# Sujit-O/pykg2vec

Measured on AMD Instinct MI355X. Metric: scored triples/sec (train) + test-triples ranked/sec, FB15k TransE d=100, higher is better.
Workload: dtype f32

## Files before the change

### include/kge_hip.h

```cpp
#ifndef KGE_HIP_H
#define KGE_HIP_H

#include <stddef.h>
#include <stdint.h>

#ifdef __cplusplus
extern "C" {
#endif

#define KGE_ABI_VERSION 3
#define KGE_MAX_TABLES 12

enum kge_model {
    KGE_TRANSE = 0,
    KGE_TRANSH = 1,
    KGE_TRANSD = 2,
    KGE_ROTATE = 3,
    KGE_RESCAL = 4,
    KGE_NTN = 5,
    KGE_DISTMULT = 6,
    KGE_COMPLEX = 7,
    KGE_ANALOGY = 8,
    KGE_TRANSM = 9,
    KGE_CP = 10,
    KGE_SIMPLE = 11,
    KGE_SIMPLE_IGNR = 12,
    KGE_QUATE = 13,
    KGE_TRANSR = 14,
    KGE_SLM = 15,
    KGE_SME = 16,
    KGE_SME_BL = 17,
    KGE_KG2E = 18,
    KGE_HOLE = 19,
    KGE_OCTONIONE = 20
};


#define KGE_FLAG_L1 1u

enum kge_optimizer { KGE_OPT_SGD = 0, KGE_OPT_ADAM = 1, KGE_OPT_ADAGRAD = 2, KGE_OPT_RMSPROP = 3,
                     KGE_OPT_GRADIENT = 4  };
enum kge_reg { KGE_REG_NONE = 0, KGE_REG_F2 = 1, KGE_REG_N3 = 2, KGE_REG_N3_ABS = 3, KGE_REG_ID_F2 = 4, KGE_REG_ID_N3 = 5 };

typedef struct kge_model_desc {
    int32_t model;
    uint32_t flags;
    int64_t tot_entity;
    int64_t tot_relation;
    int32_t dim;
    int32_t rel_dim;
    float margin;
    float phase_scale;
    const float* tables[KGE_MAX_TABLES];
    float* grads[KGE_MAX_TABLES];
} kge_model_desc;

int kge_abi_version(void);
const char* kge_last_error(void);

int kge_set_debug(int32_t check_ids);
int kge_set_switch(const char* name, int32_t value);
int kge_get_debug(void);
int kge_check_ids(const int64_t* ids, int64_t n, int64_t bound, void* stream);
size_t kge_filter_csr_workspace_bytes(int64_t n_known, int64_t n_queries);
int kge_filter_csr_count(const int64_t* known, int64_t n_known, const int64_t* queries, int64_t n_queries, int64_t tot_entity,
                         int64_t tot_relation, void* workspace, size_t workspace_bytes, int64_t* tail_off, int64_t* head_off,
                         int64_t* totals, void* stream);
int kge_filter_csr_fill(const int64_t* queries, int64_t n_queries, int64_t n_known, const void* workspace, const int64_t* tail_off,
                        const int64_t* head_off, int32_t* tail_ids, int32_t* head_ids, void* stream);

#define KGE_TOPK_MAX 1024
size_t kge_topk_workspace_bytes(int64_t nq, int64_t n_cand, int masked);
int kge_topk_rows(const void* scores, int dtype, int64_t nq, int64_t n_cand, int64_t row_stride, int32_t k, int largest,
                  const int64_t* skip_off, const int32_t* skip_ids, const int64_t* keep, void* workspace, size_t workspace_bytes,
                  int32_t* out_ids, void* out_scores, int32_t* out_count, void* stream);

#define KGE_CAND_CHUNK 64
size_t kge_rank_candidates_workspace_bytes(int64_t n, int64_t n_lists, int64_t n_cand_ids);
int kge_rank_candidates(const kge_model_desc* m, const int64_t* triples, int64_t n, int32_t side, const int64_t* list_of_query,
                        const int64_t* cand_off, const int32_t* cand_ids, int64_t n_lists, const int64_t* skip_off,
                        const int32_t* skip_ids, void* workspace, size_t workspace_bytes, int32_t* counts, void* stream);
int kge_rank_lists_from_scores(const void* scores, int dtype, const void* truth_scores, const int64_t* seg_off, int64_t n,
                               const uint8_t* flags, int largest, int32_t* counts, void* stream);

#define KGE_REL_CHUNK 64
size_t kge_rank_relations_workspace_bytes(int64_t n);
int kge_rank_relations(const kge_model_desc* m, const int64_t* triples, int64_t n, const int64_t* skip_off, const int32_t* skip_ids,
                       void* workspace, size_t workspace_bytes, int32_t* counts, void* stream);
size_t kge_relation_csr_workspace_bytes(int64_t n_known, int64_t n_queries);
int kge_relation_csr_count(const int64_t* known, int64_t n_known, const int64_t* queries, int64_t n_queries, int64_t tot_entity,
                           int64_t tot_relation, void* workspace, size_t workspace_bytes, int64_t* rel_off, int64_t* total, void* stream);
int kge_relation_csr_fill(const int64_t* queries, int64_t n_queries, int64_t n_known, const void* workspace, const int64_t* rel_off,
                          int32_t* rel_ids, void* stream);

int kge_debug_marker(int32_t tag, void* stream);

size_t kge_workspace_bytes(const kge_model_desc* m, int64_t n);

int kge_score_forward(const kge_model_desc* m, const int64_t* h, const int64_t* r, const int64_t* t,
                      int64_t n, float* scores, void* workspace, size_t workspace_bytes, void* stream);

int kge_score_backward(const kge_model_desc* m, const int64_t* h, const int64_t* r, const int64_t* t,
                       int64_t n, const float* dscore, void* workspace, size_t workspace_bytes, void* stream);

int kge_rescal_normalize(float* ent, int64_t tot_entity, float* rel, int64_t tot_relation, int32_t k,
                         void* stream);
size_t kge_rescal_normalize_scratch_bytes(int64_t tot_relation, int32_t k);
int kge_rescal_normalize_ws(float* ent , int64_t tot_entity, float* rel, int64_t tot_relation,
                            int32_t k, void* scratch, size_t scratch_bytes, void* stream);

int kge_train_pairwise_hinge(const kge_model_desc* m,
                             const int64_t* ph, const int64_t* pr, const int64_t* pt,
                             const int64_t* nh, const int64_t* nr, const int64_t* nt,
                             int64_t n, float margin, void* workspace, size_t workspace_bytes,
                             float* loss, void* stream);

int kge_train_pairwise_hinge_sampled(const kge_model_desc* m, const int64_t* triples, const int64_t* perm,
                                     int64_t start, int64_t n, const float* bern_prob, const uint64_t* slots,
                                     int64_t n_slots, uint64_t seed, uint64_t offset, const int64_t* dev_cursor,
                                     float margin, float* loss, void* stream);

int kge_train_pairwise_selfadv(const kge_model_desc* m,
                               const int64_t* ph, const int64_t* pr, const int64_t* pt,
                               const int64_t* nh, const int64_t* nr, const int64_t* nt,
                               int64_t n_pos, int32_t neg_rate, float alpha, float* workspace,
                               float* loss, void* stream);

int kge_train_pairwise_selfadv_sampled(const kge_model_desc* m, const int64_t* triples, const int64_t* perm,
                                       int64_t start, int64_t n_pos, int32_t neg_rate, float alpha,
                                       const float* bern_prob, const uint64_t* slots, int64_t n_slots,
                                       uint64_t seed, uint64_t offset, const int64_t* dev_cursor,
                                       float* loss, void* stream);

int kge_train_pointwise_logistic(const kge_model_desc* m, const int64_t* h, const int64_t* r,
                                 const int64_t* t, const int64_t* y, int64_t n,
                                 int32_t bundle ,
                                 float lmbda, int32_t reg_type, float* loss, void* stream);

int kge_train_pointwise_logistic_sampled(const kge_model_desc* m, const int64_t* triples, const int64_t* perm,
                                         int64_t start, int64_t n_pos, int32_t neg_rate, const float* bern_prob,
                                         const uint64_t* slots, int64_t n_slots, uint64_t seed, uint64_t offset,
                                         const int64_t* dev_cursor, float lmbda, int32_t reg_type, float* loss,
                                         void* stream);

int kge_optimizer_step(int32_t kind, float* param, float* grad, float* state1, float* state2,
                       int64_t numel, float lr, int64_t step, int32_t zero_grad,
                       const float* dev_hyper ,
                       void* stream);

int kge_optimizer_step_rows(int32_t kind, float* param, float* grad, float* state1, float* state2, int64_t rows, int32_t dim,
                            float lr, int64_t step, int32_t zero_grad, int32_t normalize, const float* dev_hyper,
                            const uint32_t* touched_rows, uint32_t* touched_clear, void* stream);

int kge_rescal_pair_step(const kge_model_desc* m, const int64_t* ph, const int64_t* pr, const int64_t* pt, const int64_t* nh,
                         const int64_t* nt, int64_t n, float margin, void* workspace, size_t workspace_bytes, float* loss,
                         uint32_t* touched_rows, void* stream);
int kge_rescal_pair_step_ok(const kge_model_desc* m, int64_t n);

typedef struct kge_rescal_stage {
    float* gstage;
    float* dsv;
    int32_t* count;
    int32_t* bucket;
    int32_t* head;
    int32_t* next;
    int32_t cap;
} kge_rescal_stage;
int kge_rescal_stage_ok(const kge_model_desc* m, int64_t n);
int kge_rescal_pair_step_staged(const kge_model_desc* m, const int64_t* ph, const int64_t* pr, const int64_t* pt, const int64_t* nh,
                                const int64_t* nt, int64_t n, float margin, void* workspace, size_t workspace_bytes, float* loss,
                                uint32_t* touched_rows, const kge_rescal_stage* stage, void* stream);
int kge_optimizer_step_rows_staged(int32_t kind, float* param, float* grad, float* state1, float* state2, int64_t rows, int32_t dim,
                                   float lr, int64_t step, int32_t normalize, const float* dev_hyper, const uint32_t* touched_rows,
                                   uint32_t* touched_clear, const kge_rescal_stage* stage, void* stream);

int kge_l2norm_reg(const float* param, float* grad, int64_t numel, float lmbda, float* scratch, float* loss,
                   void* stream);

size_t kge_eval_workspace_bytes(const kge_model_desc* m, int64_t n);
int kge_eval_ranks(const kge_model_desc* m, const int64_t* triples, int64_t n,
                   const int64_t* tail_off, const int32_t* tail_ids,
                   const int64_t* head_off, const int32_t* head_ids,
                   void* workspace, size_t workspace_bytes, int32_t* ranks, void* stream);

size_t kge_eval_grouped_workspace_bytes(const kge_model_desc* m, int64_t n, int64_t n_groups);
int kge_eval_ranks_grouped(const kge_model_desc* m, const int64_t* triples, int64_t n,
                           const int32_t* group_of_triple, const int64_t* group_rel, int64_t n_groups,
                           const int32_t* qblocks, int64_t n_qblocks,
                           const int64_t* tail_off, const int32_t* tail_ids,
                           const int64_t* head_off, const int32_t* head_ids,
                           void* workspace, size_t workspace_bytes, int32_t* ranks, void* stream);

int kge_eval_ranks_ties(const kge_model_desc* m, const int64_t* triples, int64_t n, const int64_t* tail_off,
                        const int32_t* tail_ids, const int64_t* head_off, const int32_t* head_ids, void* workspace,
                        size_t workspace_bytes, int32_t* ranks, int32_t* ties, void* stream);
int kge_eval_ranks_grouped_ties(const kge_model_desc* m, const int64_t* triples, int64_t n, const int32_t* group_of_triple,
                                const int64_t* group_rel, int64_t n_groups, const int32_t* qblocks, int64_t n_qblocks,
                                const int64_t* tail_off, const int32_t* tail_ids, const int64_t* head_off,
                                const int32_t* head_ids, void* workspace, size_t workspace_bytes, int32_t* ranks, int32_t* ties,
                                void* stream);

int kge_eval_sweep_scores(const kge_model_desc* m, const int64_t* triples, int64_t n,
                          void* workspace, size_t workspace_bytes, float* scores, void* stream);

int kge_eval_sweep_scores_side(const kge_model_desc* m, const int64_t* triples, int64_t n, int side,
                               void* workspace, size_t workspace_bytes, float* scores, void* stream);

int kge_rank_from_scores(const float* scores, int64_t nq, int64_t tot_entity, const int64_t* truth,
                         const int64_t* off, const int32_t* ids, int32_t* rank, int32_t* frank, void* stream);

int kge_triple_set_build(const int64_t* triples, int64_t n, uint64_t* slots, int64_t n_slots, void* stream);
int kge_corrupt(const int64_t* ph, const int64_t* pr, const int64_t* pt, int64_t n_pos, int32_t neg_rate,
                int64_t tot_entity, const float* bern_prob ,
                const uint64_t* slots, int64_t n_slots, uint64_t seed, uint64_t offset,
                int64_t* nh, int64_t* nr, int64_t* nt, void* stream);

int kge_sample_batch(const int64_t* triples, const int64_t* perm, int64_t start, int64_t n_pos, int32_t neg_rate,
                     int64_t tot_entity, const float* bern_prob, const uint64_t* slots, int64_t n_slots,
                     uint64_t seed, uint64_t offset, int32_t layout,
                     int64_t* o0, int64_t* o1, int64_t* o2, int64_t* o3, int64_t* o4, int64_t* o5,
                     const int64_t* dev_cursor ,
                     void* stream);

int kge_step_advance(int64_t* dev_cursor, float* dev_hyper, int64_t batch_stride, int64_t n_batches,
                     int64_t draws_per_batch, float lr, void* stream);

int kge_optimizer_step_rownorm_ok(int64_t rows, int64_t dim);
int kge_optimizer_step_rownorm(int32_t kind, float* param, float* grad, float* state1, float* state2, int64_t rows, int64_t dim, float lr,
                               int64_t step, int32_t zero_grad, const float* dev_hyper, void* scratch, size_t scratch_bytes,
                               const int64_t* dev_cursor, int64_t* next_cursor, float* next_hyper, int64_t batch_stride,
                               int64_t n_batches, int64_t draws_per_batch, void* stream);

int kge_optimizer_step_rows_rownorm(int32_t kind, float* param, float* grad, float* state1, float* state2, int64_t rows, int32_t dim,
                                    float* wparam, float* wgrad, float* wstate1, float* wstate2, int64_t wrows, int64_t wdim,
                                    float lr, int64_t step, int32_t zero_grad, int32_t normalize, const float* dev_hyper,
                                    const uint32_t* touched_rows, uint32_t* touched_clear, const kge_rescal_stage* stage,
                                    void* scratch, size_t scratch_bytes, const int64_t* dev_cursor, int64_t* next_cursor,
                                    float* next_hyper, int64_t batch_stride, int64_t n_batches, int64_t draws_per_batch, void* stream);

int kge_optimizer_step_advance(int32_t kind, float* param, float* grad, float* state1, float* state2,
                               int64_t numel, float lr, int32_t zero_grad,
                               const float* dev_hyper, const int64_t* dev_cursor,
                               int64_t* next_cursor, float* next_hyper,
                               int64_t batch_stride, int64_t n_batches, int64_t draws_per_batch, void* stream);

#define KGE_PULL_BUCKET 16
typedef struct kge_pull_lists {
    int32_t* pc;
    int32_t* count;
    int32_t* bucket;
    int32_t* head;
    int32_t* next;
    int32_t* sdesc;
    int32_t* dbucket;
} kge_pull_lists;
typedef struct kge_pull_direction {
    void* codes;
    float* recs;
    int64_t n_pairs;
    int32_t lists_without_descriptors;
} kge_pull_direction;
int kge_pull_direction_bytes(int32_t dim, int32_t l1, int64_t n_pairs, size_t* codes_bytes, size_t* recs_bytes);
int kge_pull_partial_stride(int32_t dim);
int kge_pull_hat_stride(int32_t dim);
int kge_pull_groups_per_block(int32_t dim);
int kge_row_norms(const float* table, int64_t rows, int32_t dim, float* norms, float* normalised, void* stream);
int kge_pull_sample(const int32_t* pairs, const int32_t* inv, int64_t n, int64_t tot_entity, const float* bern_prob,
                    const uint64_t* slots, int64_t n_slots, uint64_t seed, uint64_t offset, const int64_t* dev_cursor,
                    const kge_pull_lists* out, void* stream);
int kge_pull_lists_explicit(const int32_t* pairs, const int32_t* inv, const int64_t* nh, const int64_t* nt, int64_t n,
                            const kge_pull_lists* out, void* stream);
int kge_pull_step(const kge_model_desc* m, float* const tables_out[2], const float* const hat_in[2], float* const hat_out[2],
                  const float* norm_in, float* norm_out,
                  float* const state1[2], float* const state2[2], const int32_t* pairs, const kge_pull_lists* lists,
                  const int32_t* items, int64_t n_items, const uint32_t* dense_skip, const int32_t* inc, float* partials, const int32_t* multi,
                  int64_t n_multi, float margin, int32_t optimizer, float lr, int64_t step, const float* dev_hyper,
                  int32_t reset_lists, const int32_t* next_pairs, const int32_t* next_inv, int64_t next_n, const float* bern_prob,
                  const uint64_t* slots, int64_t n_slots, uint64_t seed, uint64_t next_offset, const kge_pull_lists* next_lists,
// ... 429 lines not shown
```

### pykg2vec_amd/_lib.py

```python
import ctypes
import os

_HERE = os.path.dirname(os.path.abspath(__file__))
LIB_PATH = os.environ.get("KGE_HIP_LIB", os.path.join(_HERE, "libkge_hip.so"))

KGE_MAX_TABLES = 12
ABI_VERSION = 3

(TRANSE, TRANSH, TRANSD, ROTATE, RESCAL, NTN, DISTMULT, COMPLEX, ANALOGY, TRANSM, CP, SIMPLE, SIMPLE_IGNR,
 QUATE, TRANSR, SLM, SME, SME_BL, KG2E, HOLE, OCTONIONE) = range(21)
FLAG_L1 = 1
OPT_SGD, OPT_ADAM, OPT_ADAGRAD, OPT_RMSPROP = range(4)
REG_NONE, REG_F2, REG_N3, REG_N3_ABS, REG_ID_F2, REG_ID_N3 = range(6)
LOSS_SLOTS, LOSS_STRIDE = 32, 32

c_i64p = ctypes.c_void_p


class ModelDesc(ctypes.Structure):
    _fields_ = [
        ("model", ctypes.c_int32),
        ("flags", ctypes.c_uint32),
        ("tot_entity", ctypes.c_int64),
        ("tot_relation", ctypes.c_int64),
# ... 197 lines not shown
_SIGNATURES = {
    **_conv_1n_signatures("interacte", InteracteDesc),
    **_conv_1n_signatures("acre", AcreDesc),
    **_conv_1n_signatures("hyper", HyperDesc),
    **_conv_1n_signatures("conve", ConveDesc, has_side=True),
    "kge_proje_body_forward_workspace_bytes": (ctypes.c_size_t, [_PJD, ctypes.c_int64]),
    "kge_proje_body_forward": (ctypes.c_int, [_PJD, ctypes.c_void_p, ctypes.c_void_p, ctypes.c_int64, ctypes.c_int32, ctypes.c_void_p,
                                              ctypes.c_void_p, ctypes.c_size_t, ctypes.c_void_p]),
    "kge_proje_body_backward_workspace_bytes": (ctypes.c_size_t, [_PJD, ctypes.c_int64]),
    "kge_proje_body_backward": (ctypes.c_int, [_PJD, ctypes.c_void_p, ctypes.c_void_p, ctypes.c_int64, ctypes.c_int32, ctypes.c_void_p,
                                               ctypes.c_void_p, ctypes.c_size_t, ctypes.c_void_p]),
    "kge_proje_label_loss_workspace_bytes": (ctypes.c_size_t, [ctypes.c_int64, ctypes.c_int32, ctypes.c_int64, ctypes.c_int64]),
    "kge_proje_label_loss": (ctypes.c_int, [ctypes.c_void_p, ctypes.c_int64, ctypes.c_int32, ctypes.c_void_p, ctypes.c_int64, ctypes.c_void_p,
                                            ctypes.c_void_p, ctypes.c_int64, ctypes.c_void_p, ctypes.c_int64, ctypes.c_void_p,
                                            ctypes.c_size_t] + [ctypes.c_void_p] * 4),
    "kge_proje_train_workspace_bytes": (ctypes.c_size_t, [_PJD] + [ctypes.c_int64] * 4),
    "kge_proje_train": (ctypes.c_int, [_PJD] + [ctypes.c_void_p] * 3 + [ctypes.c_int64, ctypes.c_void_p, ctypes.c_void_p, ctypes.c_int64,
                                                                      ctypes.c_void_p, ctypes.c_void_p, ctypes.c_int64, ctypes.c_void_p,
                                                                      ctypes.c_int64, ctypes.c_float, ctypes.c_void_p, ctypes.c_size_t,
                                                                      ctypes.c_void_p, ctypes.c_void_p]),
    "kge_proje_eval_ranks_workspace_bytes": (ctypes.c_size_t, [_PJD, ctypes.c_int64]),
    "kge_proje_eval_ranks": (ctypes.c_int, [_PJD, ctypes.c_void_p, ctypes.c_int64] + [ctypes.c_void_p] * 4
                             + [ctypes.c_void_p, ctypes.c_size_t, ctypes.c_void_p, ctypes.c_void_p, ctypes.c_void_p]),
    "kge_tucker_saved_floats": (ctypes.c_size_t, [_TKD, ctypes.c_int64]),
    "kge_tucker_body_forward_workspace_bytes": (ctypes.c_size_t, [_TKD, ctypes.c_int64]),
    "kge_tucker_body_forward": (ctypes.c_int, [_TKD, ctypes.c_void_p, ctypes.c_void_p, ctypes.c_int64, ctypes.c_void_p, ctypes.c_void_p,
                                               ctypes.c_void_p, ctypes.c_size_t, ctypes.c_void_p]),
    "kge_tucker_body_backward_workspace_bytes": (ctypes.c_size_t, [_TKD, ctypes.c_int64]),
    "kge_tucker_body_backward": (ctypes.c_int, [_TKD, ctypes.c_void_p, ctypes.c_void_p, ctypes.c_int64, ctypes.c_void_p, ctypes.c_void_p,
                                                ctypes.c_void_p, ctypes.c_size_t, ctypes.c_void_p]),
    "kge_tucker_train_bce_workspace_bytes": (ctypes.c_size_t, [_TKD, ctypes.c_int64, ctypes.c_int64, ctypes.c_int64]),
    "kge_tucker_train_bce": (ctypes.c_int, [_TKD] + [ctypes.c_void_p] * 3 + [ctypes.c_int64, ctypes.c_void_p, ctypes.c_void_p, ctypes.c_int64,
                                                                           ctypes.c_void_p, ctypes.c_void_p, ctypes.c_int64, ctypes.c_float,
                                                                           ctypes.c_void_p, ctypes.c_size_t, ctypes.c_void_p, ctypes.c_void_p]),
    "kge_tucker_eval_ranks_workspace_bytes": (ctypes.c_size_t, [_TKD, ctypes.c_int64]),
    "kge_tucker_eval_ranks": (ctypes.c_int, [_TKD, ctypes.c_void_p, ctypes.c_int64] + [ctypes.c_void_p] * 4
                              + [ctypes.c_void_p, ctypes.c_size_t, ctypes.c_void_p, ctypes.c_void_p, ctypes.c_void_p]),
    "kge_convkb_collapse_workspace_bytes": (ctypes.c_size_t, [_CKB]),
    "kge_convkb_collapse": (ctypes.c_int, [_CKB, ctypes.c_void_p, ctypes.c_void_p, ctypes.c_size_t, ctypes.c_void_p]),
    "kge_convkb_score_forward_workspace_bytes": (ctypes.c_size_t, [_CKB, ctypes.c_int64]),
    "kge_convkb_score_forward": (ctypes.c_int, [_CKB] + [ctypes.c_void_p] * 3 + [ctypes.c_int64, ctypes.c_void_p, ctypes.c_void_p,
                                                                               ctypes.c_size_t, ctypes.c_void_p]),
    "kge_convkb_score_backward_workspace_bytes": (ctypes.c_size_t, [_CKB, ctypes.c_int64]),
    "kge_convkb_score_backward": (ctypes.c_int, [_CKB] + [ctypes.c_void_p] * 3 + [ctypes.c_int64, ctypes.c_void_p, ctypes.c_void_p,
                                                                                ctypes.c_size_t, ctypes.c_void_p]),
    "kge_convkb_train_logistic_workspace_bytes": (ctypes.c_size_t, [_CKB, ctypes.c_int64]),
    "kge_convkb_train_logistic": (ctypes.c_int, [_CKB] + [ctypes.c_void_p] * 4 + [ctypes.c_int64, ctypes.c_int32, ctypes.c_void_p,
                                                                                ctypes.c_size_t, ctypes.c_void_p, ctypes.c_void_p]),
    "kge_convkb_train_logistic_sampled_workspace_bytes": (ctypes.c_size_t, [_CKB, ctypes.c_int64, ctypes.c_int32]),
    "kge_convkb_train_logistic_sampled": (ctypes.c_int, [_CKB, ctypes.c_void_p, ctypes.c_void_p, ctypes.c_int64, ctypes.c_int64,
                                                         ctypes.c_int32, ctypes.c_void_p, ctypes.c_void_p, ctypes.c_int64,
                                                         ctypes.c_uint64, ctypes.c_uint64, ctypes.c_void_p, ctypes.c_void_p,
                                                         ctypes.c_size_t, ctypes.c_void_p, ctypes.c_void_p]),
    "kge_convkb_eval_ranks_workspace_bytes": (ctypes.c_size_t, [_CKB, ctypes.c_int64]),
    "kge_convkb_eval_ranks": (ctypes.c_int, [_CKB, ctypes.c_void_p, ctypes.c_int64] + [ctypes.c_void_p] * 4
                              + [ctypes.c_void_p, ctypes.c_size_t, ctypes.c_void_p, ctypes.c_void_p]),
    "kge_convkb_sweep_scores_side_workspace_bytes": (ctypes.c_size_t, [_CKB, ctypes.c_int64]),
    "kge_murp_score_forward": (ctypes.c_int, [_MRP] + [ctypes.c_void_p] * 3 + [ctypes.c_int64, ctypes.c_void_p, ctypes.c_void_p]),
    "kge_murp_score_backward": (ctypes.c_int, [_MRP] + [ctypes.c_void_p] * 3 + [ctypes.c_int64, ctypes.c_void_p, ctypes.c_void_p]),
    "kge_murp_train_bce": (ctypes.c_int, [_MRP] + [ctypes.c_void_p] * 4 + [ctypes.c_int64, ctypes.c_void_p, ctypes.c_void_p]),
    "kge_murp_rsgd_step": (ctypes.c_int, [_MRP, ctypes.c_double, ctypes.c_int32, ctypes.c_void_p]),
    "kge_murp_eval_ranks_workspace_bytes": (ctypes.c_size_t, [_MRP, ctypes.c_int64]),
    "kge_murp_eval_ranks": (ctypes.c_int, [_MRP, ctypes.c_void_p, ctypes.c_int64] + [ctypes.c_void_p] * 4
                            + [ctypes.c_void_p, ctypes.c_size_t, ctypes.c_void_p, ctypes.c_void_p, ctypes.c_void_p]),
    "kge_murp_sweep_scores_side_workspace_bytes": (ctypes.c_size_t, [_MRP, ctypes.c_int64]),
    "kge_murp_sweep_scores_side": (ctypes.c_int, [_MRP, ctypes.c_void_p, ctypes.c_int64, ctypes.c_int32, ctypes.c_void_p,
                                                  ctypes.c_size_t, ctypes.c_void_p, ctypes.c_void_p]),
    "kge_convkb_sweep_scores_side": (ctypes.c_int, [_CKB, ctypes.c_void_p, ctypes.c_int64, ctypes.c_int32, ctypes.c_void_p,
                                                    ctypes.c_size_t, ctypes.c_void_p, ctypes.c_void_p]),
    "kge_staged_step_bytes": (ctypes.c_size_t, []),
    "kge_train_pairwise_selfadv_sampled_staged": (ctypes.c_int, [ctypes.POINTER(ModelDesc), ctypes.c_void_p, ctypes.c_void_p, ctypes.c_int64,
                                                                  ctypes.c_int64, ctypes.c_int32, ctypes.c_float, ctypes.c_void_p,
                                                                  ctypes.c_void_p, ctypes.c_int64, ctypes.c_uint64, ctypes.c_uint64,
                                                                  ctypes.POINTER(StagedStep), ctypes.c_void_p, ctypes.c_void_p]),
    "kge_train_pointwise_logistic_sampled_staged": (ctypes.c_int, [ctypes.POINTER(ModelDesc), ctypes.c_void_p, ctypes.c_void_p, ctypes.c_int64,
                                                                    ctypes.c_int64, ctypes.c_int32, ctypes.c_void_p, ctypes.c_void_p,
                                                                    ctypes.c_int64, ctypes.c_uint64, ctypes.c_uint64, ctypes.c_float,
                                                                    ctypes.c_int32, ctypes.POINTER(StagedStep), ctypes.c_void_p,
                                                                    ctypes.c_void_p]),
    "kge_optimizer_step_staged": (ctypes.c_int, [ctypes.c_int32, ctypes.POINTER(StagedStep), ctypes.c_float, ctypes.c_int64, ctypes.c_void_p]),
    "kge_abi_version": (ctypes.c_int, []),
    "kge_set_debug": (ctypes.c_int, [ctypes.c_int32]),
    "kge_set_switch": (ctypes.c_int, [ctypes.c_char_p, ctypes.c_int32]),
    "kge_get_debug": (ctypes.c_int, []),
    "kge_check_ids": (ctypes.c_int, [ctypes.c_void_p, ctypes.c_int64, ctypes.c_int64, ctypes.c_void_p]),
    "kge_debug_marker": (ctypes.c_int, [ctypes.c_int32, ctypes.c_void_p]),
    "kge_filter_csr_workspace_bytes": (ctypes.c_size_t, [ctypes.c_int64, ctypes.c_int64]),
    "kge_filter_csr_count": (ctypes.c_int, [ctypes.c_void_p, ctypes.c_int64, ctypes.c_void_p, ctypes.c_int64, ctypes.c_int64, ctypes.c_int64,
                                            ctypes.c_void_p, ctypes.c_size_t, ctypes.c_void_p, ctypes.c_void_p, ctypes.c_void_p, ctypes.c_void_p]),
    "kge_filter_csr_fill": (ctypes.c_int, [ctypes.c_void_p, ctypes.c_int64, ctypes.c_int64, ctypes.c_void_p, ctypes.c_void_p, ctypes.c_void_p,
                                           ctypes.c_void_p, ctypes.c_void_p, ctypes.c_void_p]),
    "kge_topk_workspace_bytes": (ctypes.c_size_t, [ctypes.c_int64, ctypes.c_int64, ctypes.c_int]),
    "kge_topk_rows": (ctypes.c_int, [ctypes.c_void_p, ctypes.c_int, ctypes.c_int64, ctypes.c_int64, ctypes.c_int64, ctypes.c_int32, ctypes.c_int,
                                     ctypes.c_void_p, ctypes.c_void_p, ctypes.c_void_p, ctypes.c_void_p, ctypes.c_size_t,
                                     ctypes.c_void_p, ctypes.c_void_p, ctypes.c_void_p, ctypes.c_void_p]),
    "kge_rank_candidates_workspace_bytes": (ctypes.c_size_t, [ctypes.c_int64, ctypes.c_int64, ctypes.c_int64]),
    "kge_rank_candidates": (ctypes.c_int, [ctypes.POINTER(ModelDesc), ctypes.c_void_p, ctypes.c_int64, ctypes.c_int32, ctypes.c_void_p,
                                           ctypes.c_void_p, ctypes.c_void_p, ctypes.c_int64, ctypes.c_void_p, ctypes.c_void_p,
                                           ctypes.c_void_p, ctypes.c_size_t, ctypes.c_void_p, ctypes.c_void_p]),
    "kge_rank_lists_from_scores": (ctypes.c_int, [ctypes.c_void_p, ctypes.c_int, ctypes.c_void_p, ctypes.c_void_p, ctypes.c_int64,
                                                  ctypes.c_void_p, ctypes.c_int, ctypes.c_void_p, ctypes.c_void_p]),
    "kge_rank_relations_workspace_bytes": (ctypes.c_size_t, [ctypes.c_int64]),
    "kge_rank_relations": (ctypes.c_int, [ctypes.POINTER(ModelDesc), ctypes.c_void_p, ctypes.c_int64, ctypes.c_void_p, ctypes.c_void_p,
                                          ctypes.c_void_p, ctypes.c_size_t, ctypes.c_void_p, ctypes.c_void_p]),
    "kge_relation_csr_workspace_bytes": (ctypes.c_size_t, [ctypes.c_int64, ctypes.c_int64]),
    "kge_relation_csr_count": (ctypes.c_int, [ctypes.c_void_p, ctypes.c_int64, ctypes.c_void_p, ctypes.c_int64, ctypes.c_int64, ctypes.c_int64,
                                              ctypes.c_void_p, ctypes.c_size_t, ctypes.c_void_p, ctypes.c_void_p, ctypes.c_void_p]),
    "kge_relation_csr_fill": (ctypes.c_int, [ctypes.c_void_p, ctypes.c_int64, ctypes.c_int64, ctypes.c_void_p, ctypes.c_void_p, ctypes.c_void_p,
                                             ctypes.c_void_p]),
    "kge_last_error": (ctypes.c_char_p, []),
    "kge_workspace_bytes": (ctypes.c_size_t, [ctypes.POINTER(ModelDesc), ctypes.c_int64]),
    "kge_score_forward": (ctypes.c_int, [ctypes.POINTER(ModelDesc)] + [ctypes.c_void_p] * 3 + [ctypes.c_int64, ctypes.c_void_p, ctypes.c_void_p, ctypes.c_size_t, ctypes.c_void_p]),
    "kge_score_backward": (ctypes.c_int, [ctypes.POINTER(ModelDesc)] + [ctypes.c_void_p] * 3 + [ctypes.c_int64, ctypes.c_void_p, ctypes.c_void_p, ctypes.c_size_t, ctypes.c_void_p]),
    "kge_rescal_normalize": (ctypes.c_int, [ctypes.c_void_p, ctypes.c_int64, ctypes.c_void_p, ctypes.c_int64, ctypes.c_int32, ctypes.c_void_p]),
    "kge_rescal_normalize_scratch_bytes": (ctypes.c_size_t, [ctypes.c_int64, ctypes.c_int32]),
    "kge_rescal_normalize_ws": (ctypes.c_int, [ctypes.c_void_p, ctypes.c_int64, ctypes.c_void_p, ctypes.c_int64, ctypes.c_int32, ctypes.c_void_p, ctypes.c_size_t, ctypes.c_void_p]),
    "kge_train_pairwise_hinge": (ctypes.c_int, [ctypes.POINTER(ModelDesc)] + [ctypes.c_void_p] * 6 + [ctypes.c_int64, ctypes.c_float, ctypes.c_void_p, ctypes.c_size_t, ctypes.c_void_p, ctypes.c_void_p]),
    "kge_train_pairwise_hinge_sampled": (ctypes.c_int, [ctypes.POINTER(ModelDesc), ctypes.c_void_p, ctypes.c_void_p, ctypes.c_int64, ctypes.c_int64, ctypes.c_void_p, ctypes.c_void_p, ctypes.c_int64, ctypes.c_uint64, ctypes.c_uint64, ctypes.c_void_p, ctypes.c_float, ctypes.c_void_p, ctypes.c_void_p]),
    "kge_train_pairwise_selfadv": (ctypes.c_int, [ctypes.POINTER(ModelDesc)] + [ctypes.c_void_p] * 6 + [ctypes.c_int64, ctypes.c_int32, ctypes.c_float, ctypes.c_void_p, ctypes.c_void_p, ctypes.c_void_p]),
    "kge_train_pairwise_selfadv_sampled": (ctypes.c_int, [ctypes.POINTER(ModelDesc), ctypes.c_void_p, ctypes.c_void_p, ctypes.c_int64, ctypes.c_int64, ctypes.c_int32, ctypes.c_float, ctypes.c_void_p, ctypes.c_void_p, ctypes.c_int64, ctypes.c_uint64, ctypes.c_uint64, ctypes.c_void_p, ctypes.c_void_p, ctypes.c_void_p]),
    "kge_train_pointwise_logistic": (ctypes.c_int, [ctypes.POINTER(ModelDesc)] + [ctypes.c_void_p] * 4 + [ctypes.c_int64, ctypes.c_int32, ctypes.c_float, ctypes.c_int32, ctypes.c_void_p, ctypes.c_void_p]),
    "kge_train_pointwise_logistic_sampled": (ctypes.c_int, [ctypes.POINTER(ModelDesc), ctypes.c_void_p, ctypes.c_void_p, ctypes.c_int64,
                                                            ctypes.c_int64, ctypes.c_int32, ctypes.c_void_p, ctypes.c_void_p, ctypes.c_int64,
                                                            ctypes.c_uint64, ctypes.c_uint64, ctypes.c_void_p, ctypes.c_float, ctypes.c_int32,
                                                            ctypes.c_void_p, ctypes.c_void_p]),
    "kge_l2norm_reg": (ctypes.c_int, [ctypes.c_void_p, ctypes.c_void_p, ctypes.c_int64, ctypes.c_float, ctypes.c_void_p, ctypes.c_void_p, ctypes.c_void_p]),
    "kge_head_1n_rank_workspace_bytes": (ctypes.c_size_t, [ctypes.c_int64, ctypes.c_int32, ctypes.c_int64, ctypes.c_int32]),
    "kge_head_1n_rank": (ctypes.c_int, [ctypes.c_void_p, ctypes.c_int64, ctypes.c_int32, ctypes.c_void_p, ctypes.c_int64, ctypes.c_void_p,
                                        ctypes.c_void_p, ctypes.c_void_p, ctypes.c_void_p, ctypes.c_void_p, ctypes.c_size_t,
                                        ctypes.c_void_p, ctypes.c_void_p, ctypes.c_void_p, ctypes.c_void_p]),
    "kge_head_1n_forward": (ctypes.c_int, [ctypes.c_void_p, ctypes.c_int64, ctypes.c_int32, ctypes.c_void_p, ctypes.c_int64,
                                           ctypes.c_void_p, ctypes.c_void_p, ctypes.c_void_p]),
    "kge_head_1n_forward_bf16": (ctypes.c_int, [ctypes.c_void_p, ctypes.c_int64, ctypes.c_int32, ctypes.c_void_p, ctypes.c_int64,
                                                ctypes.c_void_p, ctypes.c_void_p, ctypes.c_void_p]),
    "kge_head_1n_backward_workspace_bytes": (ctypes.c_size_t, []),
    "kge_head_1n_backward": (ctypes.c_int, [ctypes.c_void_p, ctypes.c_int64, ctypes.c_int32, ctypes.c_void_p, ctypes.c_int64]
                             + [ctypes.c_void_p] * 6 + [ctypes.c_size_t, ctypes.c_void_p]),
    "kge_head_1n_bce_workspace_bytes": (ctypes.c_size_t, [ctypes.c_int64, ctypes.c_int64, ctypes.c_int64]),
    "kge_head_1n_bce": (ctypes.c_int, [ctypes.c_void_p, ctypes.c_int64, ctypes.c_int32, ctypes.c_void_p, ctypes.c_int64,
                                       ctypes.c_void_p, ctypes.c_void_p, ctypes.c_void_p, ctypes.c_int64, ctypes.c_float,
                                       ctypes.c_void_p, ctypes.c_size_t] + [ctypes.c_void_p] * 5),
    "kge_optimizer_step": (ctypes.c_int, [ctypes.c_int32] + [ctypes.c_void_p] * 4 + [ctypes.c_int64, ctypes.c_float, ctypes.c_int64, ctypes.c_int32, ctypes.c_void_p, ctypes.c_void_p]),
    "kge_optimizer_step_rows": (ctypes.c_int, [ctypes.c_int32] + [ctypes.c_void_p] * 4 + [ctypes.c_int64, ctypes.c_int32, ctypes.c_float,
                                               ctypes.c_int64, ctypes.c_int32, ctypes.c_int32] + [ctypes.c_void_p] * 4),
    "kge_optimizer_step_rownorm_ok": (ctypes.c_int, [ctypes.c_int64, ctypes.c_int64]),
    "kge_optimizer_step_rownorm": (ctypes.c_int, [ctypes.c_int32] + [ctypes.c_void_p] * 4 + [ctypes.c_int64, ctypes.c_int64, ctypes.c_float, ctypes.c_int64,
                                                  ctypes.c_int32, ctypes.c_void_p, ctypes.c_void_p, ctypes.c_size_t, ctypes.c_void_p, ctypes.c_void_p,
                                                  ctypes.c_void_p, ctypes.c_int64, ctypes.c_int64, ctypes.c_int64, ctypes.c_void_p]),
    "kge_optimizer_step_rows_rownorm": (ctypes.c_int, [ctypes.c_int32] + [ctypes.c_void_p] * 4 + [ctypes.c_int64, ctypes.c_int32] + [ctypes.c_void_p] * 4
                                        + [ctypes.c_int64, ctypes.c_int64, ctypes.c_float, ctypes.c_int64, ctypes.c_int32, ctypes.c_int32]
                                        + [ctypes.c_void_p] * 3 + [ctypes.POINTER(RescalStage), ctypes.c_void_p, ctypes.c_size_t]
                                        + [ctypes.c_void_p] * 3 + [ctypes.c_int64] * 3 + [ctypes.c_void_p]),
    "kge_rescal_pair_step": (ctypes.c_int, [ctypes.POINTER(ModelDesc)] + [ctypes.c_void_p] * 5 + [ctypes.c_int64, ctypes.c_float, ctypes.c_void_p,
                                            ctypes.c_size_t, ctypes.c_void_p, ctypes.c_void_p, ctypes.c_void_p]),
    "kge_rescal_pair_step_ok": (ctypes.c_int, [ctypes.POINTER(ModelDesc), ctypes.c_int64]),
    "kge_rescal_stage_ok": (ctypes.c_int, [ctypes.POINTER(ModelDesc), ctypes.c_int64]),
    "kge_rescal_pair_step_staged": (ctypes.c_int, [ctypes.POINTER(ModelDesc)] + [ctypes.c_void_p] * 5 + [ctypes.c_int64, ctypes.c_float, ctypes.c_void_p,
                                                   ctypes.c_size_t, ctypes.c_void_p, ctypes.c_void_p, ctypes.POINTER(RescalStage), ctypes.c_void_p]),
    "kge_optimizer_step_rows_staged": (ctypes.c_int, [ctypes.c_int32] + [ctypes.c_void_p] * 4 + [ctypes.c_int64, ctypes.c_int32, ctypes.c_float,
                                                      ctypes.c_int64, ctypes.c_int32] + [ctypes.c_void_p] * 3 + [ctypes.POINTER(RescalStage), ctypes.c_void_p]),
    "kge_step_advance": (ctypes.c_int, [ctypes.c_void_p, ctypes.c_void_p, ctypes.c_int64, ctypes.c_int64, ctypes.c_int64, ctypes.c_float, ctypes.c_void_p]),
    "kge_optimizer_step_advance": (ctypes.c_int, [ctypes.c_int32] + [ctypes.c_void_p] * 4 + [ctypes.c_int64, ctypes.c_float, ctypes.c_int32]
                                   + [ctypes.c_void_p] * 4 + [ctypes.c_int64] * 3 + [ctypes.c_void_p]),
    "kge_eval_workspace_bytes": (ctypes.c_size_t, [ctypes.POINTER(ModelDesc), ctypes.c_int64]),
    "kge_eval_ranks": (ctypes.c_int, [ctypes.POINTER(ModelDesc), ctypes.c_void_p, ctypes.c_int64] + [ctypes.c_void_p] * 4 + [ctypes.c_void_p, ctypes.c_size_t, ctypes.c_void_p, ctypes.c_void_p]),
    "kge_eval_ranks_ties": (ctypes.c_int, [ctypes.POINTER(ModelDesc), ctypes.c_void_p, ctypes.c_int64] + [ctypes.c_void_p] * 4 + [ctypes.c_void_p, ctypes.c_size_t, ctypes.c_void_p, ctypes.c_void_p, ctypes.c_void_p]),
    "kge_eval_ranks_grouped_ties": (ctypes.c_int, [ctypes.POINTER(ModelDesc), ctypes.c_void_p, ctypes.c_int64, ctypes.c_void_p,
                                                   ctypes.c_void_p, ctypes.c_int64, ctypes.c_void_p, ctypes.c_int64]
                                    + [ctypes.c_void_p] * 4 + [ctypes.c_void_p, ctypes.c_size_t, ctypes.c_void_p, ctypes.c_void_p, ctypes.c_void_p]),
    "kge_eval_grouped_workspace_bytes": (ctypes.c_size_t, [ctypes.POINTER(ModelDesc), ctypes.c_int64, ctypes.c_int64]),
    "kge_eval_ranks_grouped": (ctypes.c_int, [ctypes.POINTER(ModelDesc), ctypes.c_void_p, ctypes.c_int64, ctypes.c_void_p,
                                              ctypes.c_void_p, ctypes.c_int64, ctypes.c_void_p, ctypes.c_int64]
                               + [ctypes.c_void_p] * 4 + [ctypes.c_void_p, ctypes.c_size_t, ctypes.c_void_p, ctypes.c_void_p]),
    "kge_eval_sweep_scores": (ctypes.c_int, [ctypes.POINTER(ModelDesc), ctypes.c_void_p, ctypes.c_int64, ctypes.c_void_p, ctypes.c_size_t, ctypes.c_void_p, ctypes.c_void_p]),
    "kge_eval_sweep_scores_side": (ctypes.c_int, [ctypes.POINTER(ModelDesc), ctypes.c_void_p, ctypes.c_int64, ctypes.c_int32, ctypes.c_void_p, ctypes.c_size_t, ctypes.c_void_p, ctypes.c_void_p]),
    "kge_rank_from_scores": (ctypes.c_int, [ctypes.c_void_p, ctypes.c_int64, ctypes.c_int64] + [ctypes.c_void_p] * 5 + [ctypes.c_void_p]),
    "kge_triple_set_build": (ctypes.c_int, [ctypes.c_void_p, ctypes.c_int64, ctypes.c_void_p, ctypes.c_int64, ctypes.c_void_p]),
    "kge_corrupt": (ctypes.c_int, [ctypes.c_void_p] * 3 + [ctypes.c_int64, ctypes.c_int32, ctypes.c_int64, ctypes.c_void_p, ctypes.c_void_p, ctypes.c_int64, ctypes.c_uint64, ctypes.c_uint64] + [ctypes.c_void_p] * 3 + [ctypes.c_void_p]),
    "kge_sample_batch": (ctypes.c_int, [ctypes.c_void_p, ctypes.c_void_p, ctypes.c_int64, ctypes.c_int64, ctypes.c_int32, ctypes.c_int64, ctypes.c_void_p, ctypes.c_void_p, ctypes.c_int64, ctypes.c_uint64, ctypes.c_uint64, ctypes.c_int32] + [ctypes.c_void_p] * 6 + [ctypes.c_void_p, ctypes.c_void_p]),
    "kge_pull_partial_stride": (ctypes.c_int, [ctypes.c_int32]),
    "kge_pull_hat_stride": (ctypes.c_int, [ctypes.c_int32]),
    "kge_pull_groups_per_block": (ctypes.c_int, [ctypes.c_int32]),
    "kge_row_norms": (ctypes.c_int, [ctypes.c_void_p, ctypes.c_int64, ctypes.c_int32, ctypes.c_void_p, ctypes.c_void_p, ctypes.c_void_p]),
    "kge_pull_sample": (ctypes.c_int, [ctypes.c_void_p, ctypes.c_void_p, ctypes.c_int64, ctypes.c_int64, ctypes.c_void_p, ctypes.c_void_p, ctypes.c_int64,
                                       ctypes.c_uint64, ctypes.c_uint64, ctypes.c_void_p, ctypes.POINTER(PullLists), ctypes.c_void_p]),
    "kge_pull_lists_explicit": (ctypes.c_int, [ctypes.c_void_p] * 4 + [ctypes.c_int64, ctypes.POINTER(PullLists), ctypes.c_void_p]),
    "kge_pull_step": (ctypes.c_int, [ctypes.POINTER(ModelDesc)] + [ctypes.c_void_p] * 8 + [ctypes.POINTER(PullLists), ctypes.c_void_p,
                                     ctypes.c_int64, ctypes.c_void_p, ctypes.c_void_p, ctypes.c_void_p, ctypes.c_void_p, ctypes.c_int64, ctypes.c_float,
                                     ctypes.c_int32, ctypes.c_float, ctypes.c_int64, ctypes.c_void_p, ctypes.c_int32,
                                     ctypes.c_void_p, ctypes.c_void_p, ctypes.c_int64, ctypes.c_void_p, ctypes.c_void_p, ctypes.c_int64,
                                     ctypes.c_uint64, ctypes.c_uint64, ctypes.POINTER(PullLists), ctypes.c_void_p,
                                     ctypes.POINTER(PullDirection), ctypes.c_void_p]),
    "kge_pull_direction_bytes": (ctypes.c_int, [ctypes.c_int32, ctypes.c_int32, ctypes.c_int64, ctypes.POINTER(ctypes.c_size_t),
                                                ctypes.POINTER(ctypes.c_size_t)]),
    "kge_transx_groups_per_block": (ctypes.c_int, [ctypes.c_int32]),
    "kge_transx_partial_stride": (ctypes.c_int, [ctypes.c_int32]),
    "kge_transx_scratch_bytes": (ctypes.c_int, [ctypes.c_int32, ctypes.c_int32, ctypes.c_int64, ctypes.POINTER(ctypes.c_size_t),
                                                ctypes.POINTER(ctypes.c_size_t)]),
    "kge_transx_grad_step": (ctypes.c_int, [ctypes.POINTER(ModelDesc), ctypes.c_void_p, ctypes.c_int64, ctypes.POINTER(PullLists), ctypes.c_void_p,
                                            ctypes.c_int64, ctypes.c_void_p, ctypes.c_void_p, ctypes.c_void_p, ctypes.c_void_p, ctypes.c_int64,
                                            ctypes.c_float, ctypes.c_void_p, ctypes.c_void_p, ctypes.c_int32,
                                            ctypes.c_void_p, ctypes.c_void_p, ctypes.c_int64, ctypes.c_void_p, ctypes.c_void_p, ctypes.c_int64,
                                            ctypes.c_uint64, ctypes.c_uint64, ctypes.POINTER(PullLists), ctypes.c_void_p, ctypes.c_void_p]),
    "kge_transx_plan_bytes": (ctypes.c_size_t, []),
    "kge_transx_run": (ctypes.c_int, [ctypes.POINTER(TransXPlanC), ctypes.c_int64, ctypes.c_int64, ctypes.c_int32, ctypes.c_int32,
                                      ctypes.c_int64, ctypes.c_uint64, ctypes.c_int32, ctypes.c_void_p]),
    "kge_own_groups_per_block": (ctypes.c_int, [ctypes.c_int32, ctypes.c_int32]),
    "kge_own_partial_stride": (ctypes.c_int, [ctypes.c_int32, ctypes.c_int32]),
    "kge_own_stage_bytes": (ctypes.c_size_t, [ctypes.c_int32, ctypes.c_int32, ctypes.c_int64]),
    "kge_own_step": (ctypes.c_int, [ctypes.POINTER(ModelDesc), ctypes.c_void_p, ctypes.c_int64, ctypes.POINTER(PullLists), ctypes.c_void_p,
                                    ctypes.c_int64, ctypes.c_void_p, ctypes.c_void_p, ctypes.c_void_p, ctypes.c_int32, ctypes.c_float,
                                    ctypes.c_int32, ctypes.c_int32, ctypes.c_void_p, ctypes.c_void_p, ctypes.c_int64, ctypes.c_void_p,
                                    ctypes.c_void_p, ctypes.c_int64, ctypes.c_uint64, ctypes.c_uint64, ctypes.POINTER(PullLists),
                                    ctypes.c_void_p, ctypes.c_void_p, ctypes.c_void_p]),
    "kge_own_apply": (ctypes.c_int, [ctypes.POINTER(ModelDesc), ctypes.c_void_p, ctypes.c_void_p, ctypes.c_void_p, ctypes.c_int64,
                                     ctypes.POINTER(PullLists), ctypes.c_void_p, ctypes.c_int64, ctypes.c_void_p, ctypes.c_void_p,
                                     ctypes.c_int64, ctypes.c_void_p, ctypes.c_int32, ctypes.c_int32, ctypes.c_float, ctypes.c_int64,
                                     ctypes.c_void_p]),
    "kge_own_plan_bytes": (ctypes.c_size_t, []),
    "kge_own_run": (ctypes.c_int, [ctypes.POINTER(OwnPlanC), ctypes.c_int64, ctypes.c_int64, ctypes.c_int32, ctypes.c_int32,
                                   ctypes.c_int64, ctypes.c_uint64, ctypes.c_int32, ctypes.c_void_p]),
    "kge_pull_index_geometry": (ctypes.c_int, [ctypes.c_int64] * 4 + [ctypes.c_int32] * 3 + [ctypes.POINTER(ctypes.c_int64)] * 3
                                + [ctypes.POINTER(ctypes.c_size_t)]),
    "kge_pull_index_build": (ctypes.c_int, [ctypes.c_void_p, ctypes.c_void_p] + [ctypes.c_int64] * 6 + [ctypes.c_int32] * 3
                             + [ctypes.c_void_p] * 8 + [ctypes.c_size_t, ctypes.c_void_p]),
    "kge_pull_plan_bytes": (ctypes.c_size_t, []),
    "kge_pull_run": (ctypes.c_int, [ctypes.POINTER(PullPlanC), ctypes.c_int64, ctypes.c_int64, ctypes.c_int32, ctypes.c_int32,
                                    ctypes.c_int32, ctypes.c_int64, ctypes.c_uint64, ctypes.c_int32, ctypes.c_void_p]),
}
EXPORTED_SYMBOLS = tuple(_SIGNATURES)

_lib = None


class KgeHipError(RuntimeError):
    pass


def load():
    global _lib
    if _lib is not None:
        return _lib
    if not os.path.exists(LIB_PATH):
        raise KgeHipError("libkge_hip.so not found at %s -- the HIP extension is mandatory (no CPU fallback); "
                          "run __graft_entry__.build()" % LIB_PATH)
    lib = ctypes.CDLL(LIB_PATH)
    for name, (res, args) in _SIGNATURES.items():
        fn = getattr(lib, name)
        fn.restype = res
# ... 12 lines not shown
```

### pykg2vec_amd/csrc/kge_api.hip

```cpp
#include <stdarg.h>
#include <stdio.h>
#include <string.h>
#include <cstdlib>
#include "kge_internal.h"

namespace kge {

static thread_local char g_err[512] = "";

void set_error(const char* fmt, ...) {
    va_list ap;
    va_start(ap, fmt);
    vsnprintf(g_err, sizeof(g_err), fmt, ap);
    va_end(ap);
}

static bool is_vector_model(int model) { return model_ops(model)->row_kernels; }

bool pick_geometry(int d, Geometry* out) {
    if (d <= 0) return false;
    if (d <= 32) *out = {32, 1};
    else if (d <= 64) *out = {32, 2};
    else if (d <= 128) *out = {32, 4};
    else if (d <= 256) *out = {32, 8};
// ... 712 lines not shown
        }
        int rc = kge_own_step(&p->model, b->pairs, b->n_pairs, &p->lists[cl], b->items, b->n_items, b->dense_skip, b->inc, p->partials,
                              dense, p->lmbda, p->reg_type, 1, next_pairs, next_inv, next_n, p->bern_prob, p->slots, p->n_slots, p->seed,
                              next_offset, next_lists, p->loss, nullptr, stream);
        if (rc) return rc;
        return kge_own_apply(&p->model, p->state1, p->state2, b->pairs, b->n_pairs, &p->lists[cl], b->items, b->n_items, b->dense_skip,
                             b->multi, b->n_multi, p->partials, dense, p->optimizer, p->lr, first_opt_step + k, stream);
    });
}

int kge_head_1n_forward(const float* x, int64_t batch, int32_t dim, const float* ent, int64_t tot_entity, const float* bias,
                        float* preds, void* stream) {
    return launch_head_forward(x, batch, dim, ent, tot_entity, bias, preds, 0, (hipStream_t)stream);
}

int kge_head_1n_forward_bf16(const float* x, int64_t batch, int32_t dim, const float* ent, int64_t tot_entity, const float* bias,
                             float* preds, void* stream) {
    return launch_head_forward(x, batch, dim, ent, tot_entity, bias, preds, 1, (hipStream_t)stream);
}

size_t kge_head_1n_rank_workspace_bytes(int64_t batch, int32_t dim, int64_t tot_entity, int32_t has_bias) {
    if (batch < 0 || dim <= 0 || tot_entity <= 0) return 0;
    return head_rank_workspace_bytes(batch, dim, tot_entity, has_bias != 0);
}

int kge_head_1n_rank(const float* x, int64_t batch, int32_t dim, const float* ent, int64_t tot_entity, const float* bias,
                     const int64_t* triples, const int64_t* off, const int32_t* ids, void* workspace, size_t workspace_bytes,
                     int32_t* ranks, int32_t* ties, float* energies, void* stream) {
    if (batch == 0) return 0;
    if (batch < 0 || dim <= 0 || tot_entity <= 0 || !x || !ent || !triples || (!ranks && !energies) || ((off == nullptr) != (ids == nullptr))) {
        set_error("kge_head_1n_rank: bad arguments");
        return -1;
    }
    if (tot_entity >= (1ll << 31)) { set_error("kge_head_1n_rank: entity ids must fit 31 bits"); return -1; }
    if (int rc = debug_check_ids("kge_head_1n_rank", "true entity", triples, batch, 3, 2, tot_entity, (hipStream_t)stream)) return rc;
    return launch_head_rank(x, batch, dim, ent, tot_entity, bias, triples, off, ids, workspace, workspace_bytes, ranks, ties, energies,
                            (hipStream_t)stream);
}

size_t kge_head_1n_backward_workspace_bytes(void) { return head_backward_workspace_bytes(); }

int kge_head_1n_backward(const float* x, int64_t batch, int32_t dim, const float* ent, int64_t tot_entity, const float* preds,
                         const float* dpreds, float* dx, float* g_ent, float* g_bias, void* workspace, size_t workspace_bytes,
                         void* stream) {
    return launch_head_backward(x, batch, dim, ent, tot_entity, preds, dpreds, dx, g_ent, g_bias, workspace, workspace_bytes,
                                (hipStream_t)stream);
}

size_t kge_head_1n_bce_workspace_bytes(int64_t batch, int64_t tot_entity, int64_t n_pos) {
    if (batch <= 0 || tot_entity <= 0 || n_pos < 0) return 0;
    return head_bce_workspace_bytes(batch, tot_entity, n_pos);
}

int kge_head_1n_bce(const float* x, int64_t batch, int32_t dim, const float* ent, int64_t tot_entity, const float* bias,
                    const int64_t* label_off, const int32_t* label_ids, int64_t n_pos, float label_smoothing,
                    void* workspace, size_t workspace_bytes, float* loss, float* dx, float* g_ent, float* g_bias,
                    void* stream) {
    return launch_head_bce(x, batch, dim, ent, tot_entity, bias, label_off, label_ids, n_pos, label_smoothing, workspace,
                           workspace_bytes, loss, dx, g_ent, g_bias, (hipStream_t)stream);
}

int kge_l2norm_reg(const float* param, float* grad, int64_t numel, float lmbda, float* scratch, float* loss, void* stream) {
    if (!param || !grad || !scratch || !loss || numel <= 0) { set_error("kge_l2norm_reg: bad arguments"); return -1; }
    return launch_l2norm_reg(param, grad, numel, lmbda, scratch, loss, (hipStream_t)stream);
}

size_t kge_eval_workspace_bytes(const kge_model_desc* m, int64_t n) {
    if (validate(m, false, "kge_eval_workspace_bytes") || n < 0) return 0;
    return eval_workspace_bytes(m, n);
}

int kge_eval_ranks_ties(const kge_model_desc* m, const int64_t* triples, int64_t n, const int64_t* tail_off,
                        const int32_t* tail_ids, const int64_t* head_off, const int32_t* head_ids, void* workspace,
                        size_t workspace_bytes, int32_t* ranks, int32_t* ties, void* stream) {
    if (validate(m, false, "kge_eval_ranks")) return -1;
    if (n == 0) return 0;
    if (n < 0 || !triples || !ranks) { set_error("kge_eval_ranks: bad arguments"); return -1; }
    if ((tail_off && !tail_ids) || (head_off && !head_ids)) { set_error("kge_eval_ranks: CSR offsets without ids"); return -1; }
    if (int rc = debug_check_triples("kge_eval_ranks", m->tot_entity, m->tot_relation, triples, n, (hipStream_t)stream)) return rc;
    return launch_eval_ranks(m, triples, n, tail_off, tail_ids, head_off, head_ids, workspace, workspace_bytes, ranks, ties,
                             (hipStream_t)stream);
}

int kge_eval_ranks(const kge_model_desc* m, const int64_t* triples, int64_t n, const int64_t* tail_off,
                   const int32_t* tail_ids, const int64_t* head_off, const int32_t* head_ids, void* workspace,
                   size_t workspace_bytes, int32_t* ranks, void* stream) {
    return kge_eval_ranks_ties(m, triples, n, tail_off, tail_ids, head_off, head_ids, workspace, workspace_bytes, ranks, nullptr, stream);
}

size_t kge_eval_grouped_workspace_bytes(const kge_model_desc* m, int64_t n, int64_t n_groups) {
    if (validate(m, false, "kge_eval_grouped_workspace_bytes") || n < 0 || n_groups < 1) return 0;
    return eval_workspace_bytes(m, n, n_groups == 1 ? 2 : n_groups);
}

int kge_eval_ranks_grouped_ties(const kge_model_desc* m, const int64_t* triples, int64_t n, const int32_t* group_of_triple,
                                const int64_t* group_rel, int64_t n_groups, const int32_t* qblocks, int64_t n_qblocks,
                                const int64_t* tail_off, const int32_t* tail_ids, const int64_t* head_off,
                                const int32_t* head_ids, void* workspace, size_t workspace_bytes, int32_t* ranks, int32_t* ties,
                                void* stream) {
    if (validate(m, false, "kge_eval_ranks_grouped")) return -1;
    if (n == 0) return 0;
    if (n < 0 || !triples || !ranks || !group_of_triple || !group_rel || !qblocks || n_groups < 1 || n_qblocks < 1) {
        set_error("kge_eval_ranks_grouped: bad arguments");
        return -1;
    }
    if ((tail_off && !tail_ids) || (head_off && !head_ids)) { set_error("kge_eval_ranks_grouped: CSR offsets without ids"); return -1; }
    if (int rc = debug_check_triples("kge_eval_ranks_grouped", m->tot_entity, m->tot_relation, triples, n, (hipStream_t)stream)) return rc;
    return launch_eval_ranks_grouped(m, triples, n, group_of_triple, group_rel, n_groups, qblocks, n_qblocks, tail_off, tail_ids,
                                     head_off, head_ids, workspace, workspace_bytes, ranks, ties, (hipStream_t)stream);
}

int kge_eval_ranks_grouped(const kge_model_desc* m, const int64_t* triples, int64_t n, const int32_t* group_of_triple,
                           const int64_t* group_rel, int64_t n_groups, const int32_t* qblocks, int64_t n_qblocks,
                           const int64_t* tail_off, const int32_t* tail_ids, const int64_t* head_off,
                           const int32_t* head_ids, void* workspace, size_t workspace_bytes, int32_t* ranks, void* stream) {
    return kge_eval_ranks_grouped_ties(m, triples, n, group_of_triple, group_rel, n_groups, qblocks, n_qblocks, tail_off, tail_ids,
                                       head_off, head_ids, workspace, workspace_bytes, ranks, nullptr, stream);
}

int kge_eval_sweep_scores(const kge_model_desc* m, const int64_t* triples, int64_t n, void* workspace,
                          size_t workspace_bytes, float* scores, void* stream) {
    if (validate(m, false, "kge_eval_sweep_scores")) return -1;
    if (n == 0) return 0;
    if (n < 0 || !triples || !scores) { set_error("kge_eval_sweep_scores: bad arguments"); return -1; }
    if (int rc = debug_check_triples("kge_eval_sweep_scores", m->tot_entity, m->tot_relation, triples, n, (hipStream_t)stream)) return rc;
    return launch_eval_sweep_scores(m, triples, n, workspace, workspace_bytes, scores, (hipStream_t)stream);
}

int kge_eval_sweep_scores_side(const kge_model_desc* m, const int64_t* triples, int64_t n, int side, void* workspace,
                               size_t workspace_bytes, float* scores, void* stream) {
    if (validate(m, false, "kge_eval_sweep_scores_side")) return -1;
    if (n == 0) return 0;
    if (n < 0 || !triples || !scores || (side != 0 && side != 1)) { set_error("kge_eval_sweep_scores_side: bad arguments (side is 0 = tail sweep or 1 = head sweep)"); return -1; }
    if (int rc = debug_check_triples("kge_eval_sweep_scores_side", m->tot_entity, m->tot_relation, triples, n, (hipStream_t)stream)) return rc;
    return launch_eval_sweep_scores(m, triples, n, workspace, workspace_bytes, scores, (hipStream_t)stream, side);
}

int kge_rank_from_scores(const float* scores, int64_t nq, int64_t tot_entity, const int64_t* truth, const int64_t* off,
                         const int32_t* ids, int32_t* rank, int32_t* frank, void* stream) {
    if (nq == 0) return 0;
    if (!scores || !truth || !rank || !frank || nq < 0 || tot_entity <= 0 || (off && !ids)) {
        set_error("kge_rank_from_scores: bad arguments");
        return -1;
    }
    if (int rc = debug_check_ids("kge_rank_from_scores", "true entity", truth, nq, 1, 0, tot_entity, (hipStream_t)stream)) return rc;
    return launch_rank_from_scores(scores, nq, tot_entity, truth, off, ids, rank, frank, (hipStream_t)stream);
}

int kge_triple_set_build(const int64_t* triples, int64_t n, uint64_t* slots, int64_t n_slots, void* stream) {
    if (!triples || !slots || n < 0 || n_slots < 2 * n || (n_slots & (n_slots - 1))) {
        set_error("kge_triple_set_build: n_slots must be a power of two >= 2n");
        return -1;
    }
    if (int rc = debug_check_triples("kge_triple_set_build", (int64_t)1 << 24, (int64_t)1 << 16, triples, n, (hipStream_t)stream)) return rc;
    return launch_triple_set_build(triples, n, slots, n_slots, (hipStream_t)stream);
}

int kge_corrupt(const int64_t* ph, const int64_t* pr, const int64_t* pt, int64_t n_pos, int32_t neg_rate,
                int64_t tot_entity, const float* bern_prob, const uint64_t* slots, int64_t n_slots, uint64_t seed,
                uint64_t offset, int64_t* nh, int64_t* nr, int64_t* nt, void* stream) {
    if (n_pos == 0) return 0;
    if (!ph || !pr || !pt || !nh || !nr || !nt || n_pos < 0 || neg_rate <= 0 || tot_entity <= 1) {
        set_error("kge_corrupt: bad arguments");
        return -1;
    }
    if (slots && (n_slots & (n_slots - 1))) { set_error("kge_corrupt: n_slots must be a power of two"); return -1; }
// ... 37 lines not shown
```

### pykg2vec_amd/csrc/kge_debug.hip

```cpp
#include <cstdlib>
#include <cstring>
#include <cstdio>
#include "kge_internal.h"

namespace kge {

struct SwitchOverride { char name[32]; int value; };
static SwitchOverride g_overrides[16];
static int g_n_overrides = 0;

int switch_value(const char* name) {
    for (int i = 0; i < g_n_overrides; ++i)
        if (!strcmp(g_overrides[i].name, name)) { if (g_overrides[i].value >= 0) return g_overrides[i].value; break; }
    char var[48];
    snprintf(var, sizeof(var), "KGE_%s", name);
    const char* e = getenv(var);
    if (!e || !e[0]) return -1;
    return atoi(e);
}
static int set_switch(const char* name, int value) {
    for (int i = 0; i < g_n_overrides; ++i)
        if (!strcmp(g_overrides[i].name, name)) { g_overrides[i].value = value; return 0; }
    if (g_n_overrides == 16 || strlen(name) >= sizeof(g_overrides[0].name)) return -1;
    strcpy(g_overrides[g_n_overrides].name, name);
    g_overrides[g_n_overrides++].value = value;
    return 0;
}

static int g_debug = -1;

bool debug_ids() {
    if (g_debug < 0) {
        const char* e = getenv("KGE_DEBUG_IDS");
        g_debug = (e && e[0] && e[0] != '0') ? 1 : 0;
    }
    return g_debug > 0;
}
void set_debug_ids(int on) { g_debug = on ? 1 : 0; }

struct BadId { unsigned long long pos; long long value; };

__global__ __launch_bounds__(256) void k_check_ids(const int64_t* __restrict__ ids, const int64_t* __restrict__ perm, int64_t start,
                                                   int64_t n, int stride, int col, int64_t bound, unsigned long long* __restrict__ first,
                                                   long long* __restrict__ value) {
    for (int64_t i = (int64_t)blockIdx.x * blockDim.x + threadIdx.x; i < n; i += (int64_t)gridDim.x * blockDim.x) {
        const int64_t row = perm ? perm[start + i] : i;
        const int64_t v = ids[row * stride + col];
        if (v < 0 || v >= bound) {
            const unsigned long long old = atomicMin(first, (unsigned long long)i);
            if ((unsigned long long)i < old) *value = v;
        }
    }
}
__global__ void k_check_ids32(const int32_t* __restrict__ ids, int64_t n, int stride, int col, int64_t bound,
                              unsigned long long* __restrict__ first, long long* __restrict__ value) {
    for (int64_t i = (int64_t)blockIdx.x * blockDim.x + threadIdx.x; i < n; i += (int64_t)gridDim.x * blockDim.x) {
        const int64_t v = ids[i * stride + col];
        if (v < 0 || v >= bound) {
            const unsigned long long old = atomicMin(first, (unsigned long long)i);
            if ((unsigned long long)i < old) *value = v;
        }
    }
}

__global__ void k_check_ascending(const int64_t* __restrict__ off, const int32_t* __restrict__ ids, int64_t n,
                                  unsigned long long* __restrict__ first, long long* __restrict__ value) {
    for (int64_t i = (int64_t)blockIdx.x * blockDim.x + threadIdx.x; i < n; i += (int64_t)gridDim.x * blockDim.x) {
        for (int64_t j = off[i] + 1; j < off[i + 1]; ++j) {
            if (ids[j] < ids[j - 1]) {
                const unsigned long long old = atomicMin(first, (unsigned long long)j);
                if ((unsigned long long)j < old) *value = ids[j];
                break;
            }
        }
    }
}

static BadId* g_flag = nullptr;

static bool capturing(hipStream_t s) {
    hipStreamCaptureStatus st = hipStreamCaptureStatusNone;
    if (hipStreamIsCapturing(s, &st) != hipSuccess) { (void)hipGetLastError(); return false; }
    return st != hipStreamCaptureStatusNone;
}

static int run_check(const char* who, const char* what, int64_t bound, hipStream_t s, void (*launch)(void*, BadId*, hipStream_t), void* ctx) {
    if (capturing(s)) return 0;
    if (!g_flag && hipMalloc(&g_flag, sizeof(BadId)) != hipSuccess) { set_error("%s: debug id check: hipMalloc failed", who); return -2; }
    BadId init{~0ull, 0};
    if (hipMemcpyAsync(g_flag, &init, sizeof(init), hipMemcpyHostToDevice, s) != hipSuccess) { set_error("%s: debug id check: copy failed", who); return -2; }
    launch(ctx, g_flag, s);
    BadId out;
    if (hipMemcpyAsync(&out, g_flag, sizeof(out), hipMemcpyDeviceToHost, s) != hipSuccess || hipStreamSynchronize(s) != hipSuccess) {
        set_error("%s: debug id check failed to run: %s", who, hipGetErrorString(hipGetLastError()));
        return -2;
    }
    if (out.pos != ~0ull && bound < 0) {
        set_error("%s: %s segments must be ascending: id %lld at position %llu is below its predecessor", who, what, out.value, out.pos);
        return -3;
    }
    if (out.pos != ~0ull) {
        set_error("%s: %s id out of range at position %llu: %lld not in [0, %lld) (an nn.Embedding lookup would raise IndexError, "
                  "models/Domain.py:8-13)", who, what, out.pos, out.value, (long long)bound);
        return -3;
    }
    return 0;
// ... 79 lines not shown
```

### pykg2vec_amd/csrc/kge_eval.hip

```cpp
#include "kge_internal.h"
#include <stdlib.h>
#include <string.h>

namespace kge {

#ifndef KGE_GEMM_CHUNK
#define KGE_GEMM_CHUNK 64
#endif
constexpr int kGemmChunk = KGE_GEMM_CHUNK;
constexpr int KC = 8;
constexpr int QT_PLAIN = 16;
constexpr int QT_XF = 8;

enum Form { F_L1 = 0, F_L2 = 1, F_SQM = 2, F_NEGDOT = 3 };
enum XForm { X_NONE = 0, X_TRANSH = 1, X_TRANSD = 2 };
enum Post { P_NONE = 0, P_SCALE = 1, P_CLAMP = 2, P_SIGMOID = 3 };

struct EvalPlan {
    int64_t nq;
    int only;
    int64_t E, n, tables, table_stride;
    int K, Kpad, QV, form, xform, post;
    int64_t ntiles;
    float* cand; float* aux; float* qvec; float* qscale; float* st; int32_t* fcount; int32_t* rcount; int32_t* tcount;
    float* qT;
    size_t bytes;
};

static int sweep_K(const kge_model_desc* m) {
    switch (m->model) {
        case KGE_COMPLEX: case KGE_ROTATE: case KGE_ANALOGY: return 2 * m->dim;
        case KGE_CP: case KGE_SIMPLE: case KGE_SIMPLE_IGNR: return 2 * m->dim;
        case KGE_QUATE: return 4 * m->dim;
        case KGE_TRANSR: return m->rel_dim;
        case KGE_HEAD_1N_INTERNAL: return m->dim + (m->tables[1] ? 1 : 0);
        default: return m->dim;
    }
}

static bool make_plan(const kge_model_desc* m, int64_t n, void* ws, EvalPlan* p, int64_t tables = 1) {
    p->E = m->tot_entity; p->n = n; p->nq = 2 * n; p->only = 2; p->tables = tables;
    const bool per_group_tables = tables > 1 || m->model == KGE_TRANSR;
    p->K = sweep_K(m);
    p->Kpad = (p->K + KC - 1) / KC * KC;
    p->xform = per_group_tables ? X_NONE : m->model == KGE_TRANSH ? X_TRANSH : m->model == KGE_TRANSD ? X_TRANSD : X_NONE;
    p->QV = p->xform == X_NONE ? 1 : 2;
    switch (m->model) {
        case KGE_TRANSE: case KGE_TRANSH: case KGE_TRANSD: case KGE_TRANSM: case KGE_TRANSR:
            p->form = (m->flags & KGE_FLAG_L1) ? F_L1 : F_L2; break;
        case KGE_ROTATE: p->form = F_SQM; break;
        case KGE_DISTMULT: case KGE_COMPLEX: case KGE_ANALOGY: case KGE_RESCAL:
        case KGE_CP: case KGE_SIMPLE: case KGE_SIMPLE_IGNR: case KGE_QUATE: case KGE_HEAD_1N_INTERNAL: case KGE_DOT_INTERNAL: p->form = F_NEGDOT; break;
        default: return false;
    }
    p->post = m->model == KGE_TRANSM ? P_SCALE : (m->model == KGE_SIMPLE || m->model == KGE_SIMPLE_IGNR) ? P_CLAMP
              : (m->model == KGE_HEAD_1N_INTERNAL || (m->model == KGE_DOT_INTERNAL && (m->flags & kDotSigmoid))) ? P_SIGMOID : P_NONE;
    p->ntiles = (p->E + 63) / 64;
    const bool dot_form = (p->form == F_NEGDOT || p->form == F_SQM) && p->xform == X_NONE;
    if (dot_form) p->Kpad = (p->K + 15) / 16 * 16;
    size_t off = 0;
    char* base = (char*)ws;
    auto take = [&](size_t bytes) { char* q = base ? base + off : nullptr; off += align256(bytes); return q; };
    p->table_stride = p->ntiles * p->Kpad * 64;
    p->cand = (float*)take(((size_t)tables * p->table_stride + (dot_form ? (size_t)p->Kpad * 64 : 0)) * sizeof(float));
    p->aux = (float*)take((size_t)p->ntiles * 64 * sizeof(float));
    p->qvec = (float*)take((size_t)2 * n * p->QV * p->Kpad * sizeof(float));
    p->qscale = (float*)take((size_t)2 * n * sizeof(float));
    p->st = (float*)take((size_t)2 * n * sizeof(float));
    p->fcount = (int32_t*)take((size_t)2 * n * sizeof(int32_t));
    p->rcount = (int32_t*)take((size_t)4 * n * sizeof(int32_t));
    p->tcount = p->rcount ? p->rcount + 2 * n : nullptr;
    p->qT = nullptr;
    if ((p->form == F_NEGDOT || p->form == F_SQM) && p->xform == X_NONE)
        p->qT = (float*)take((size_t)((2 * n + 127) / 128) * p->Kpad * 128 * sizeof(float));
    p->bytes = off;
    return true;
}

size_t eval_workspace_bytes(const kge_model_desc* m, int64_t n, int64_t tables) {
    if (WsBytesFn* own = model_ops(m->model)->eval_ws) return own(m, n);
    EvalPlan p;
    if (!make_plan(m, n, nullptr, &p, tables)) return 0;
    return p.bytes;
}

struct PrepArgs {
    const float* seg[4]; int seg_dim[4]; int nseg;
    const float* dot_tab;
    int normalize;
    int want_n2;
    int64_t E; int K, Kpad;
    int kper;
};

__device__ __forceinline__ float prep_elem(const PrepArgs& a, int64_t e, int k) {
    int kk = k;
#pragma unroll
    for (int s = 0; s < 4; ++s) {
        if (s < a.nseg) {
            if (kk < a.seg_dim[s]) return a.seg[s][e * a.seg_dim[s] + kk];
            kk -= a.seg_dim[s];
        }
    }
    return 0.f;
}

__device__ __forceinline__ const float* prep_addr(const PrepArgs& a, int64_t e, int k) {
    const float* ptr = nullptr;
    int kk = k;
#pragma unroll
    for (int s = 0; s < 4; ++s) {
        if (s < a.nseg) {
            const bool in = kk >= 0 && kk < a.seg_dim[s];
            ptr = in ? a.seg[s] + e * a.seg_dim[s] + kk : ptr;
            kk -= a.seg_dim[s];
        }
    }
    return ptr;
}

__global__ __launch_bounds__(256) void k_eval_prepare(PrepArgs a, float* __restrict__ cand, float* __restrict__ aux) {
    __shared__ float s_scale[64];
    __shared__ float s_tile[64][65];
    const int lane = threadIdx.x & 63, wave = threadIdx.x >> 6;
    const int64_t tile = blockIdx.x;
    const int64_t e0 = tile * 64;
    if (a.normalize) {
        for (int j = 0; j < 16; ++j) {
            const int row = wave * 16 + j;
            const int64_t e = e0 + row;
            float n2 = 0.f;
            if (e < a.E)
                for (int k = lane; k < a.K; k += 64) { const float v = prep_elem(a, e, k); n2 = fmaf(v, v, n2); }
            n2 = wave_sum(n2);
            if (lane == 0) s_scale[row] = 1.0f / fmaxf(sqrtf(n2), kEpsNormalize);
        }
    } else if (threadIdx.x < 64) {
        s_scale[threadIdx.x] = 1.0f;
    }
    __syncthreads();
    float n2acc[16], dtacc[16];
#pragma unroll
    for (int j = 0; j < 16; ++j) { n2acc[j] = 0.f; dtacc[j] = 0.f; }
    const int k_lo = blockIdx.y * a.kper, k_hi = min(a.Kpad, k_lo + a.kper);
    for (int k0 = k_lo; k0 < k_hi; k0 += 64) {
#pragma unroll
        for (int j = 0; j < 16; ++j) {
            const int row = wave * 16 + j;
            const int64_t e = e0 + row;
            const int k = k0 + lane;
            float v = 0.f;
            if (e < a.E && k < a.K) {
                const float raw = prep_elem(a, e, k);
                if (a.want_n2) n2acc[j] = fmaf(raw, raw, n2acc[j]);
                if (a.dot_tab) dtacc[j] = fmaf(raw, a.dot_tab[e * a.K + k], dtacc[j]);
                v = raw * s_scale[row];
            }
// ... 599 lines not shown
                    for (int u = 0; u < 4; ++u) {
                        c4[u] = *reinterpret_cast<const float4*>(cr + kk + 4 * u);
                        q4[u] = *reinterpret_cast<const float4*>(sq + kk + 4 * u);
                    }
#pragma unroll
                    for (int u = 0; u < 4; ++u) {
                        acc = fmaf(c4[u].x, q4[u].x, acc); acc = fmaf(c4[u].y, q4[u].y, acc);
                        acc = fmaf(c4[u].z, q4[u].z, acc); acc = fmaf(c4[u].w, q4[u].w, acc);
                    }
                    if (kGemmChunk && ((k0 + kk + 16) % (kGemmChunk ? kGemmChunk : 1)) == 0) { tot += acc; acc = 0.f; }
                }
                for (; kk < nk; kk += 8) {
                    const float4 c0 = *reinterpret_cast<const float4*>(cr + kk), c1 = *reinterpret_cast<const float4*>(cr + kk + 4);
                    const float4 q0 = *reinterpret_cast<const float4*>(sq + kk), q1 = *reinterpret_cast<const float4*>(sq + kk + 4);
                    acc = fmaf(c0.x, q0.x, acc); acc = fmaf(c0.y, q0.y, acc); acc = fmaf(c0.z, q0.z, acc); acc = fmaf(c0.w, q0.w, acc);
                    acc = fmaf(c1.x, q1.x, acc); acc = fmaf(c1.y, q1.y, acc); acc = fmaf(c1.z, q1.z, acc); acc = fmaf(c1.w, q1.w, acc);
                    if (kGemmChunk && ((k0 + kk + 8) % (kGemmChunk ? kGemmChunk : 1)) == 0) { tot += acc; acc = 0.f; }
                }
            }
            __builtin_amdgcn_wave_barrier();
        }
        if (kGemmChunk) acc = tot + acc;
        if constexpr (FORM == F_SQM) acc = sqm_from_dot(acc, qn, lane < pg ? aux[e] : 0.f);
        const float sco = pair_post<POST>(pair_finish<FORM>(acc, margin), 1.0f);
        if (base == 0) s_true = __shfl(sco, 0, 64);
        if (lane < pg && idx > 0 && e != truth) cnt += (sco < s_true) ? 1 : 0;
        base += pg;
    }
    cnt = (int)wave_sum((float)cnt);
    if (lane == 0) { st[qi] = s_true; fcount[qi] = cnt; }
}

typedef float f32x2 __attribute__((ext_vector_type(2)));

template <int FORM>
__device__ __forceinline__ void pair_step2(float& acc, f32x2 c, f32x2 q) {
    if constexpr (FORM == F_NEGDOT) {
        acc = fmaf(c.x, q.x, acc);
        acc = fmaf(c.y, q.y, acc);
    } else if constexpr (FORM == F_L1) {
        acc = add_abs(acc, c.x - q.x);
        acc = add_abs(acc, c.y - q.y);
    } else {
        const f32x2 d = c - q;
        acc = fma_sq(acc, d.x); acc = fma_sq(acc, d.y);
    }
}

template <int QT, int NS, class F>
__device__ __forceinline__ void for_query_chunks(const float* const (&qrow)[QT], const int (&off)[NS], F body) {
    float nx[NS][KC];
#pragma unroll
    for (int s = 0; s < NS; ++s)
#pragma unroll
        for (int j = 0; j < KC; ++j) nx[s][j] = qrow[0][off[s] + j];
#pragma unroll
    for (int q = 0; q < QT; ++q) {
        float cur[NS][KC];
#pragma unroll
        for (int s = 0; s < NS; ++s)
#pragma unroll
            for (int j = 0; j < KC; ++j) cur[s][j] = nx[s][j];
#pragma unroll
        for (int s = 0; s < NS; ++s) asm volatile("" ::"s"(cur[s][0]), "s"(cur[s][KC - 1]));
        if (q + 1 < QT) {
#pragma unroll
            for (int s = 0; s < NS; ++s)
#pragma unroll
                for (int j = 0; j < KC; ++j) nx[s][j] = qrow[q + 1][off[s] + j];
        }
        __builtin_amdgcn_sched_barrier(0);
        body(q, cur);
        __builtin_amdgcn_sched_barrier(0);
    }
}

template <int FORM, int XFORM, int QT, bool WRITE, int POST>
__global__ __launch_bounds__(256) void k_eval_sweep(const float* __restrict__ cand, const float* __restrict__ aux,
                                                    const float* __restrict__ qvec, const float* __restrict__ qscale,
                                                    const float* __restrict__ st,
                                                    int64_t nq, int64_t E, int64_t ntiles, int Kpad, int QV, float margin,
                                                    int S, int qblocks, int32_t* __restrict__ rcount,
                                                    int32_t* __restrict__ tcount, float* __restrict__ scores_out,
                                                    const int32_t* __restrict__ qdesc, int64_t table_stride) {
    const int lane = threadIdx.x & 63;
    const int wave = threadIdx.x >> 6;
    const int slot = blockIdx.x & 255;
    const int mm = blockIdx.x >> 8;
    const int ts = mm % S;
    const int qb = (mm / S) * 256 + slot;
    if (qb >= qblocks) return;
    int64_t q0 = (int64_t)qb * QT;
    if (qdesc) {
        cand += qdesc[4 * qb] * table_stride;
        q0 = qdesc[4 * qb + 1];
        nq = q0 + qdesc[4 * qb + 2];
    }
    const int64_t qstride = (int64_t)QV * Kpad;
    const float* qrow[QT];
    float sthr[QT];
    float qsc[QT];
    int cnt[QT];
    int tie[QT];
#pragma unroll
    for (int q = 0; q < QT; ++q) {
        const int64_t qi = (q0 + q < nq) ? q0 + q : nq - 1;
        qrow[q] = qvec + qi * qstride;
        sthr[q] = WRITE ? 0.f : st[qi];
        qsc[q] = POST == P_SCALE ? qscale[qi] : 1.0f;
        cnt[q] = 0;
        tie[q] = 0;
    }
    if constexpr (XFORM == X_NONE) {
        for (int64_t tile = ((int64_t)ts * 4 + wave) * 2; tile < ntiles; tile += (int64_t)S * 8) {
            const bool has_b = tile + 1 < ntiles;
            const float* ca = cand + (tile * Kpad) * 64 + lane;
            const float* cb = has_b ? ca + (int64_t)Kpad * 64 : ca;
            float acca[QT], accb[QT];
            f32x2 pa[QT], pb[QT];
#pragma unroll
            for (int q = 0; q < QT; ++q) { acca[q] = 0.f; accb[q] = 0.f; pa[q] = f32x2{0.f, 0.f}; pb[q] = f32x2{0.f, 0.f}; }
            for (int k0 = 0; k0 < Kpad; k0 += KC) {
                f32x2 va[KC / 2], vb[KC / 2];
#pragma unroll
                for (int j = 0; j < KC / 2; ++j) {
                    va[j].x = ca[(int64_t)(k0 + 2 * j) * 64]; va[j].y = ca[(int64_t)(k0 + 2 * j + 1) * 64];
                    vb[j].x = cb[(int64_t)(k0 + 2 * j) * 64]; vb[j].y = cb[(int64_t)(k0 + 2 * j + 1) * 64];
                }
                const int off1[1] = {k0};
                for_query_chunks<QT, 1>(qrow, off1, [&](int q, const float (&qv)[1][KC]) {
#pragma unroll
                    for (int j = 0; j < KC / 2; ++j) {
                        f32x2 qq;
                        qq.x = qv[0][2 * j];
                        qq.y = qv[0][2 * j + 1];
                        if constexpr (FORM == F_NEGDOT) {
                            pa[q] = __builtin_elementwise_fma(va[j], qq, pa[q]);
                            pb[q] = __builtin_elementwise_fma(vb[j], qq, pb[q]);
                        } else if constexpr (FORM == F_L2 || FORM == F_SQM) {
                            const f32x2 da = va[j] - qq, db = vb[j] - qq;
                            pa[q] = __builtin_elementwise_fma(da, da, pa[q]);
                            pb[q] = __builtin_elementwise_fma(db, db, pb[q]);
                        } else {
                            pair_step2<FORM>(acca[q], va[j], qq);
                            pair_step2<FORM>(accb[q], vb[j], qq);
                        }
                    }
                });
            }
            if constexpr (FORM != F_L1) {
#pragma unroll
                for (int q = 0; q < QT; ++q) { acca[q] = pa[q].x + pa[q].y; accb[q] = pb[q].x + pb[q].y; }
            }
            const int64_t ea = tile * 64 + lane, eb = ea + 64;
            const bool valid_a = ea < E, valid_b = has_b && eb < E;
#pragma unroll
            for (int q = 0; q < QT; ++q) {
                const float sa = pair_post<POST>(pair_finish<FORM>(acca[q], margin), qsc[q]);
                const float sb = pair_post<POST>(pair_finish<FORM>(accb[q], margin), qsc[q]);
                if constexpr (WRITE) {
                    if (q0 + q < nq) {
                        if (valid_a) scores_out[(q0 + q) * E + ea] = sa;
                        if (valid_b) scores_out[(q0 + q) * E + eb] = sb;
                    }
                } else {
                    cnt[q] += __popcll(__ballot(valid_a && sa < sthr[q])) + __popcll(__ballot(valid_b && sb < sthr[q]));
                    tie[q] += __popcll(__ballot(valid_a && sa == sthr[q])) + __popcll(__ballot(valid_b && sb == sthr[q]));
// ... 2 lines not shown
        }
    } else {
    for (int64_t tile = (int64_t)ts * 4 + wave; tile < ntiles; tile += (int64_t)S * 4) {
        const float* c = cand + (tile * Kpad) * 64 + lane;
        float acc[QT];
#pragma unroll
        for (int q = 0; q < QT; ++q) acc[q] = 0.f;
        {
            float p[QT], inv[QT];
            if constexpr (XFORM == X_TRANSH) {
#pragma unroll
                for (int q = 0; q < QT; ++q) p[q] = 0.f;
                for (int k0 = 0; k0 < Kpad; k0 += KC) {
                    float cv[KC];
#pragma unroll
                    for (int j = 0; j < KC; ++j) cv[j] = c[(int64_t)(k0 + j) * 64];
                    const int off1[1] = {Kpad + k0};
                    for_query_chunks<QT, 1>(qrow, off1, [&](int q, const float (&qv)[1][KC]) {
#pragma unroll
                        for (int j = 0; j < KC; ++j) p[q] = fmaf(cv[j], qv[0][j], p[q]);
                    });
                }
#pragma unroll
                for (int q = 0; q < QT; ++q) p[q] = -p[q];
            } else {
                const float a_e = aux[tile * 64 + lane];
#pragma unroll
                for (int q = 0; q < QT; ++q) p[q] = a_e;
            }
#pragma unroll
            for (int q = 0; q < QT; ++q) inv[q] = 0.f;
            for (int k0 = 0; k0 < Kpad; k0 += KC) {
                float cv[KC];
#pragma unroll
                for (int j = 0; j < KC; ++j) cv[j] = c[(int64_t)(k0 + j) * 64];
                const int off1[1] = {Kpad + k0};
                for_query_chunks<QT, 1>(qrow, off1, [&](int q, const float (&qv)[1][KC]) {
#pragma unroll
                    for (int j = 0; j < KC; ++j) {
                        const float v = fmaf(p[q], qv[0][j], cv[j]);
                        inv[q] = fmaf(v, v, inv[q]);
                    }
                });
            }
#pragma unroll
            for (int q = 0; q < QT; ++q) inv[q] = 1.0f / fmaxf(sqrtf(inv[q]), kEpsNormalize);
            for (int k0 = 0; k0 < Kpad; k0 += KC) {
                float cv[KC];
#pragma unroll
                for (int j = 0; j < KC; ++j) cv[j] = c[(int64_t)(k0 + j) * 64];
                const int off2[2] = {Kpad + k0, k0};
                for_query_chunks<QT, 2>(qrow, off2, [&](int q, const float (&qv)[2][KC]) {
#pragma unroll
                    for (int j = 0; j < KC; ++j) {
                        const float v = fmaf(p[q], qv[0][j], cv[j]) * inv[q];
                        acc[q] = pair_step<FORM>(acc[q], v, qv[1][j]);
                    }
                });
            }
        }
        const int64_t e = tile * 64 + lane;
        const bool valid = e < E;
#pragma unroll
        for (int q = 0; q < QT; ++q) {
            const float s = pair_post<POST>(pair_finish<FORM>(acc[q], margin), qsc[q]);
            if constexpr (WRITE) {
                if (valid && q0 + q < nq) scores_out[(q0 + q) * E + e] = s;
            } else {
                cnt[q] += __popcll(__ballot(valid && s < sthr[q]));
                tie[q] += __popcll(__ballot(valid && s == sthr[q]));
            }
        }
    }
    }
    if constexpr (!WRITE) {
        if (lane == 0) {
#pragma unroll
            for (int q = 0; q < QT; ++q) {
                if (q0 + q < nq && cnt[q] != 0) atomicAdd(rcount + q0 + q, cnt[q]);
                if (tcount && q0 + q < nq && tie[q] != 0) atomicAdd(tcount + q0 + q, tie[q]);
            }
        }
    }
}

typedef float f32x16 __attribute__((ext_vector_type(16)));
constexpr int GT = 128;
#ifndef KGE_GEMM_KS
#define KGE_GEMM_KS 16
#endif
constexpr int GKS = KGE_GEMM_KS;
constexpr int GNJ = GKS / 8;
static_assert(kGemmChunk % GKS == 0, "the running total is folded at K slab boundaries");
#if defined(KGE_GEMM_32X32) && KGE_GEMM_CHUNK
#error "the 32x32x2 experiment form of k_eval_gemm keeps the single chain: build it with -DKGE_GEMM_CHUNK=0"
#endif
#ifdef KGE_GEMM_32X32
constexpr int GLD = GT + 4;
#else
constexpr int GLD = GT + 16;
#endif

__global__ __launch_bounds__(256) void k_eval_qt(const float* __restrict__ qvec, int64_t nq, int Kpad, float* __restrict__ qT) {
    __shared__ float s_t[64][65];
    const int64_t q0 = (int64_t)blockIdx.x * 64;
    const int k0 = blockIdx.y * 64;
    const int tx = threadIdx.x & 63, ty = threadIdx.x >> 6;
    for (int r = ty; r < 64; r += 4) {
        const int64_t q = q0 + r;
        s_t[r][tx] = (q < nq && k0 + tx < Kpad) ? qvec[q * Kpad + k0 + tx] : 0.f;
    }
    __syncthreads();
    for (int r = ty; r < 64; r += 4) {
        const int k = k0 + r;
        const int64_t q = q0 + tx;
        if (k < Kpad) qT[((q / GT) * Kpad + k) * GT + (q % GT)] = s_t[tx][r];
    }
}

__global__ __launch_bounds__(256) void k_eval_qnorm(const float* __restrict__ qvec, int64_t nq, int Kpad, float* __restrict__ qn) {
    const int lane = threadIdx.x & 63;
    const int64_t q = (int64_t)blockIdx.x * 4 + (threadIdx.x >> 6);
    if (q >= nq) return;
    float n2 = 0.f;
    for (int k = lane; k < Kpad; k += 64) { const float v = qvec[q * Kpad + k]; n2 = fmaf(v, v, n2); }
    n2 = wave_sum(n2);
    if (lane == 0) qn[q] = n2;
}

struct GemmSplit { int xcd, a, S, m; };
static GemmSplit gemm_split(int qtiles, int64_t ctiles, int slots_per_xcd, unsigned* grid, int S_flat) {
    GemmSplit g{0, 0, 0, 0};
    const int sw = switch_value("EVAL_GEMM_XCD");
    if (sw == 0) { *grid = (unsigned)(qtiles * S_flat); return g; }
    const int a = qtiles / 8, r = qtiles % 8;
    const int smax = (int)(ctiles < slots_per_xcd ? ctiles : slots_per_xcd);
    for (int S = smax; S >= 1; --S) {
        int m = 0;
        if (r) {
            m = a ? (S + 7) / 8 : (int)((ctiles + 7) / 8 < slots_per_xcd / r ? (ctiles + 7) / 8 : slots_per_xcd / r);
            if (m < 1) m = 1;
        }
        if (a * S + r * m <= slots_per_xcd || S == 1) {
            g.xcd = 1; g.a = a; g.S = a ? S : 0; g.m = m;
            *grid = (unsigned)(8 * (g.a * g.S + r * m));
            return g;
        }
    }
    *grid = (unsigned)(qtiles * S_flat);
    return g;
}

template <bool WRITE, int POST, bool SQM>
#ifndef KGE_GEMM_OCC
#define KGE_GEMM_OCC (kGemmChunk > 0 ? 2 : SQM ? 3 : 4)
#endif
__global__ __launch_bounds__(256, KGE_GEMM_OCC) void k_eval_gemm(const float* __restrict__ cand, const float* __restrict__ qT,
                                                   const float* __restrict__ st, int64_t nq, int64_t E, int64_t ntiles64,
                                                   int Kpad, int qtiles, int S, GemmSplit gs, int32_t* __restrict__ rcount,
                                                   int32_t* __restrict__ tcount, float* __restrict__ scores_out, const float* __restrict__ qn,
                                                   const float* __restrict__ cn, float margin) {
    __shared__ float sA[2][GKS][GLD], sB[2][GKS][GLD];
    const int lane = threadIdx.x & 63, wave = threadIdx.x >> 6;
    const int wr = wave >> 1, wc = wave & 1;
    const int64_t ctiles = (ntiles64 + 1) / 2;
    int qt, ct0, cstride;
// ... 166 lines not shown
#pragma unroll
        for (int kk = 0; kk < GKS; kk += 4) {
            float a4[4], b4[4];
#pragma unroll
            for (int i = 0; i < 4; ++i) { a4[i] = na[i]; b4[i] = nb[i]; }
            if (kk + 4 < GKS) KGE_GEMM_READ(kk + 4)
            KGE_KEEP_READS_AHEAD();
            if (kGemmChunk > 0 && kk == 0 && c_first) {
                const f32x4 zero = {0.f, 0.f, 0.f, 0.f};
#pragma unroll
                for (int mi = 0; mi < 4; ++mi)
#pragma unroll
                    for (int ni = 0; ni < 4; ++ni) acc[mi][ni] = __builtin_amdgcn_mfma_f32_16x16x4f32(a4[mi], b4[ni], zero, 0, 0, 0);
            } else {
#pragma unroll
                for (int mi = 0; mi < 4; ++mi)
#pragma unroll
                    for (int ni = 0; ni < 4; ++ni) acc[mi][ni] = __builtin_amdgcn_mfma_f32_16x16x4f32(a4[mi], b4[ni], acc[mi][ni], 0, 0, 0);
            }
        }
        if (c_last) {
#pragma unroll
            for (int mi = 0; mi < 4; ++mi)
#pragma unroll
                for (int ni = 0; ni < 4; ++ni) tot[mi][ni] += acc[mi][ni];
        }
        if (++cu_sl != nslab) return;
        cu_sl = 0;
        const int64_t ct = cu_ct;
        cu_ct += cstride;
        const int e_base = (int)(ct * GT) + wr * 64 + 16 * lk4;
        const int e_lim = (int)E;
        const bool full = ct * GT + GT <= E && (ct * 2 + 1 < ntiles64);
        const int e_pad = (int)(ntiles64 * 64);
#pragma unroll
        for (int mi = 0; mi < 4; ++mi)
#pragma unroll
            for (int reg = 0; reg < 4; ++reg) {
                const int e = e_base + 4 * reg + mi;
                float cn2 = 0.f;
                if constexpr (SQM) cn2 = e < e_pad ? cn[e] : 0.f;
#pragma unroll
                for (int ni = 0; ni < 4; ++ni) {
                    const float sc = energy(kGemmChunk > 0 ? tot[mi][ni][reg] : acc[mi][ni][reg], ni, cn2);
                    if constexpr (WRITE) {
                        const int64_t q = (int64_t)qt * GT + qcol(ni);
                        if (q < nq && e < e_lim) scores_out[q * E + e] = sc;
                    } else {
                        cnt[ni] += (sc < thr[ni] && (full || e < e_lim)) ? 1 : 0;
                        tcnt[ni] += (sc == thr[ni] && (full || e < e_lim)) ? 1 : 0;
                    }
                }
            }
#pragma unroll
        for (int mi = 0; mi < 4; ++mi)
#pragma unroll
            for (int ni = 0; ni < 4; ++ni) {
                if constexpr (kGemmChunk > 0) tot[mi][ni] = f32x4{0.f, 0.f, 0.f, 0.f};
                else acc[mi][ni] = f32x4{0.f, 0.f, 0.f, 0.f};
            }
    };
    for (int64_t g = 0; g < nsteps; g += 2) {
        body(std::integral_constant<int, 0>{}, g);
        if (g + 1 < nsteps) body(std::integral_constant<int, 1>{}, g + 1);
    }
    if constexpr (!WRITE) {
#pragma unroll
        for (int ni = 0; ni < 4; ++ni) {
            int c2 = cnt[ni] + __shfl_xor(cnt[ni], 16, 64);
            c2 += __shfl_xor(c2, 32, 64);
            int t2 = tcnt[ni] + __shfl_xor(tcnt[ni], 16, 64);
            t2 += __shfl_xor(t2, 32, 64);
            const int64_t q = (int64_t)qt * GT + qcol(ni);
            if (lk4 == 0 && q < nq && c2 != 0) atomicAdd(rcount + q, c2);
            if (tcount && lk4 == 0 && q < nq && t2 != 0) atomicAdd(tcount + q, t2);
        }
    }
}
#undef KGE_GEMM_READ

#endif

__global__ void k_eval_finalize(const int32_t* __restrict__ rcount, const int32_t* __restrict__ fcount, int64_t n,
                                int32_t* __restrict__ ranks, const int32_t* __restrict__ tcount, int32_t* __restrict__ ties) {
    const int64_t i = (int64_t)blockIdx.x * blockDim.x + threadIdx.x;
    if (i >= n) return;
    if (ties) {
        ties[i] = max(0, tcount[2 * i + 1] - 1);
        ties[n + i] = max(0, tcount[2 * i] - 1);
    }
    const int32_t rt = rcount[2 * i], rh = rcount[2 * i + 1];
    ranks[i] = rh;
    ranks[n + i] = rt;
    ranks[2 * n + i] = rh - fcount[2 * i + 1];
    ranks[3 * n + i] = rt - fcount[2 * i];
}

__global__ void k_eval_finalize_side(const int32_t* __restrict__ rcount, const int32_t* __restrict__ fcount, int64_t n,
                                     int32_t* __restrict__ ranks, const int32_t* __restrict__ tcount, int32_t* __restrict__ ties) {
    const int64_t i = (int64_t)blockIdx.x * blockDim.x + threadIdx.x;
    if (i >= n) return;
    if (ties) ties[i] = max(0, tcount[i] - 1);
    ranks[i] = rcount[i];
    ranks[n + i] = rcount[i] - fcount[i];
}

__global__ __launch_bounds__(256) void k_rank_from_scores(const float* __restrict__ scores, int64_t nq, int64_t E,
                                                          const int64_t* __restrict__ truth, const int64_t* __restrict__ off,
                                                          const int32_t* __restrict__ ids, int32_t* __restrict__ rank,
                                                          int32_t* __restrict__ frank) {
    const int lane = threadIdx.x & 63;
    const int64_t q = (int64_t)blockIdx.x * 4 + (threadIdx.x >> 6);
    if (q >= nq) return;
    const float* s = scores + q * E;
    const int64_t tr = truth[q];
    const float st = s[tr];
    int cnt = 0, fc = 0;
    for (int64_t e = lane; e < E; e += 64) cnt += s[e] < st ? 1 : 0;
    if (off) {
        for (int64_t j = off[q] + lane; j < off[q + 1]; j += 64) {
            const int64_t e = ids[j];
            fc += (e != tr && s[e] < st) ? 1 : 0;
        }
    }
    cnt = (int)wave_sum((float)cnt);
    fc = (int)wave_sum((float)fc);
    if (lane == 0) { rank[q] = cnt; frank[q] = cnt - fc; }
}

int launch_rank_from_scores(const float* scores, int64_t nq, int64_t E, const int64_t* truth, const int64_t* off,
                            const int32_t* ids, int32_t* rank, int32_t* frank, hipStream_t s) {
    hipLaunchKernelGGL(k_rank_from_scores, dim3((unsigned)((nq + 3) / 4)), dim3(256), 0, s, scores, nq, E, truth, off, ids, rank,
                       frank);
    return check_launch("k_rank_from_scores");
}

static void fill_prep(const kge_model_desc* m, const EvalPlan& p, PrepArgs* a) {
    a->nseg = 1; a->dot_tab = nullptr; a->normalize = 0; a->want_n2 = 0;
    a->E = p.E; a->K = p.K; a->Kpad = p.Kpad;
    for (int s = 0; s < 4; ++s) { a->seg[s] = nullptr; a->seg_dim[s] = 0; }
    a->seg[0] = m->tables[0]; a->seg_dim[0] = m->dim;
    switch (m->model) {
        case KGE_TRANSE: case KGE_TRANSM: a->normalize = 1; break;
        case KGE_CP:
            a->nseg = 2; a->seg[1] = m->tables[2]; a->seg_dim[1] = m->dim; break;
        case KGE_SIMPLE: case KGE_SIMPLE_IGNR:
            a->nseg = 2; a->seg[0] = m->tables[1]; a->seg[1] = m->tables[0]; a->seg_dim[1] = m->dim; break;
        case KGE_QUATE:
            a->nseg = 4;
            for (int q = 1; q < 4; ++q) { a->seg[q] = m->tables[q]; a->seg_dim[q] = m->dim; }
            break;
        case KGE_TRANSD: a->dot_tab = m->tables[2]; break;
        case KGE_COMPLEX: case KGE_ROTATE:
            a->nseg = 2; a->seg[1] = m->tables[1]; a->seg_dim[1] = m->dim; break;
        case KGE_ANALOGY:
            a->nseg = 3; a->seg[1] = m->tables[2]; a->seg_dim[1] = m->dim / 2;
            a->seg[2] = m->tables[3]; a->seg_dim[2] = m->dim / 2; break;
        case KGE_HEAD_1N_INTERNAL:
            if (m->tables[1]) { a->nseg = 2; a->seg[1] = m->tables[1]; a->seg_dim[1] = 1; }
            break;
        default: break;
    }
}

static bool use_gemm_sweep(const EvalPlan& p, int64_t nq) {
    const int force = switch_value("EVAL_GEMM");
    if (force >= 0) return force == 1;
    return nq >= 512 && p.Kpad >= 32;
}

template <int FORM, int XFORM, int POST = P_NONE>
static void launch_tf_and_sweep(const EvalPlan& p, const kge_model_desc* m, const int64_t* triples,
                                const int64_t* tail_off, const int32_t* tail_ids, const int64_t* head_off,
                                const int32_t* head_ids, float* scores_out, hipStream_t s,
                                const int32_t* group_of_triple = nullptr, const int32_t* qdesc = nullptr,
                                int64_t n_qblocks = 0) {
    constexpr int QT = XFORM == X_NONE ? QT_PLAIN : QT_XF;
    const int64_t nq = p.nq;
    const int qblocks = qdesc ? (int)n_qblocks : (int)((nq + QT - 1) / QT);
    const int64_t tiles_per_wave_pass = XFORM == X_NONE ? 2 : 1;
    const int64_t max_split = (p.ntiles + 4 * tiles_per_wave_pass - 1) / (4 * tiles_per_wave_pass);
    const int64_t qgroups = (qblocks + 255) / 256;
    int64_t S = (48 + qgroups - 1) / qgroups;
    if (S > max_split) S = max_split;
    if (S < 1) S = 1;
    const unsigned grid = (unsigned)(qgroups * 256 * S);
    if constexpr ((FORM == F_NEGDOT || FORM == F_SQM) && XFORM == X_NONE && POST != P_SCALE) {
        if (qdesc == nullptr && p.qT != nullptr && p.Kpad % GKS == 0 && use_gemm_sweep(p, nq)) {
            constexpr bool SQM = FORM == F_SQM;
            const int qtiles = (int)((nq + GT - 1) / GT);
            const int64_t ctiles = (p.ntiles + 1) / 2;
            int64_t S2 = ((KGE_GEMM_OCC) * 256) / qtiles;
            if (S2 > ctiles) S2 = ctiles;
            if (S2 < 1) S2 = 1;
            unsigned ggrid = 0;
            const GemmSplit gs = gemm_split(qtiles, ctiles, (KGE_GEMM_OCC) * 32, &ggrid, (int)S2);
            hipLaunchKernelGGL(k_eval_qt, dim3((unsigned)(qtiles * 2), (unsigned)((p.Kpad + 63) / 64)), dim3(256), 0, s, p.qvec, nq,
                               p.Kpad, p.qT);
            if (SQM)
                hipLaunchKernelGGL(k_eval_qnorm, dim3((unsigned)((nq + 3) / 4)), dim3(256), 0, s, p.qvec, nq, p.Kpad, p.qscale);
            if (scores_out == nullptr) {
                PrepArgs pa;
                fill_prep(m, p, &pa);
                hipLaunchKernelGGL((k_eval_target_filter_chain<FORM, POST>), dim3((unsigned)((nq + 3) / 4)), dim3(256), 0, s, pa, p.aux,
                                   p.qvec, p.qscale, triples, p.n, p.Kpad, m->margin, tail_off, tail_ids, head_off, head_ids, p.st,
                                   p.fcount, p.only);
                hipLaunchKernelGGL((k_eval_gemm<false, POST, SQM>), dim3(ggrid), dim3(256), 0, s, p.cand, p.qT, p.st,
                                   nq, p.E, p.ntiles, p.Kpad, qtiles, (int)S2, gs, p.rcount, p.tcount, nullptr, p.qscale, p.aux, m->margin);
            } else {
                hipLaunchKernelGGL((k_eval_gemm<true, POST, SQM>), dim3(ggrid), dim3(256), 0, s, p.cand, p.qT, p.st,
                                   nq, p.E, p.ntiles, p.Kpad, qtiles, (int)S2, gs, p.rcount, nullptr, scores_out, p.qscale, p.aux, m->margin);
            }
            return;
        }
    }
    if (scores_out == nullptr)
        hipLaunchKernelGGL((k_eval_target_filter<FORM, XFORM, POST>), dim3((unsigned)((nq + 3) / 4)), dim3(256), 0, s, p.cand,
                           p.aux, p.qvec, p.qscale, triples, p.n, p.Kpad, p.QV, m->margin, tail_off, tail_ids, head_off, head_ids,
                           p.st, p.fcount, group_of_triple, p.table_stride, p.only);
    if (scores_out == nullptr) {
        hipLaunchKernelGGL((k_eval_sweep<FORM, XFORM, QT, false, POST>), dim3(grid), dim3(256), 0, s, p.cand, p.aux, p.qvec,
                           p.qscale, p.st, nq, p.E, p.ntiles, p.Kpad, p.QV, m->margin, (int)S, qblocks, p.rcount, p.tcount, nullptr,
                           qdesc, p.table_stride);
    } else {
        hipLaunchKernelGGL((k_eval_sweep<FORM, XFORM, QT, true, POST>), dim3(grid), dim3(256), 0, s, p.cand, p.aux, p.qvec,
                           p.qscale, p.st, nq, p.E, p.ntiles, p.Kpad, p.QV, m->margin, (int)S, qblocks, p.rcount, nullptr, scores_out,
                           qdesc, p.table_stride);
    }
}

static int run_pipeline(const kge_model_desc* m, const int64_t* triples, int64_t n, const int64_t* tail_off,
                        const int32_t* tail_ids, const int64_t* head_off, const int32_t* head_ids, void* ws,
                        size_t ws_bytes, int32_t* ranks, int32_t* ties, float* scores_out, hipStream_t s, int side) {
    EvalPlan p;
    if (!make_plan(m, n, ws, &p)) { set_error("kge_eval: model %d has no sweep form", m->model); return -1; }
    if (side != 2) {
        if ((side != 0 && side != 1) || m->model == KGE_TRANSR) {
            set_error("kge_eval: one-sided sweeps take side 0 = tail or 1 = head (TransR projects per call: use both sides)");
            return -1;
        }
        p.nq = n;
        p.only = side;
    }
    if (ws == nullptr || ws_bytes < p.bytes) {
        set_error("kge_eval: workspace too small (%zu < %zu)", ws_bytes, p.bytes);
        return -1;
    }
    if (n <= 0) return 0;
    if (m->model == KGE_TRANSR) {
        int rc = launch_transr_eval_prepare(m, triples, n, nullptr, 1, p.Kpad, p.ntiles, p.cand, p.qvec, p.qscale, s);
        if (rc) return rc;
    } else {
    PrepArgs pa;
    fill_prep(m, p, &pa);
    pa.want_n2 = (p.form == F_SQM && p.xform == X_NONE && p.qT != nullptr && use_gemm_sweep(p, p.nq)) ? 1 : 0;
    bool vec = !pa.normalize && !pa.dot_tab;
    for (int sg = 0; sg < pa.nseg; ++sg) vec = vec && pa.seg_dim[sg] % 4 == 0 && (uintptr_t)pa.seg[sg] % 16 == 0;
    if (vec) {
        const int64_t nchunks = (p.Kpad + 127) / 128;
        int64_t nky = min(nchunks, (2048 + p.ntiles - 1) / p.ntiles);
        if (pa.want_n2 && nky > 1) {
            const int64_t cap = (int64_t)((2 * n + 127) / 128) * p.Kpad * 128 / (p.ntiles * 64);
            if (cap < nky) nky = cap;
        }
        if (nky < 1) nky = 1;
        pa.kper = (int)((nchunks + nky - 1) / nky * 128);
        nky = (p.Kpad + pa.kper - 1) / pa.kper;
        float* part = (pa.want_n2 && nky > 1) ? p.qT : nullptr;
        hipLaunchKernelGGL(k_eval_prepare4, dim3((unsigned)p.ntiles, (unsigned)nky), dim3(256), 0, s, pa, p.cand, p.aux, part);
        if (part)
            hipLaunchKernelGGL(k_eval_cnorm_parts, dim3((unsigned)((p.ntiles * 64 + 255) / 256)), dim3(256), 0, s, part, (int)nky,
                               p.ntiles * 64, p.aux);
    } else {
    int ksplit = 1;
    if (!pa.normalize && !pa.dot_tab) {
        ksplit = (int)min((int64_t)((p.Kpad + 63) / 64), (4096 + p.ntiles - 1) / p.ntiles);
        if (ksplit < 1) ksplit = 1;
    }
    pa.kper = ((p.Kpad + ksplit - 1) / ksplit + 63) / 64 * 64;
    ksplit = (p.Kpad + pa.kper - 1) / pa.kper;
    hipLaunchKernelGGL(k_eval_prepare, dim3((unsigned)p.ntiles, (unsigned)ksplit), dim3(256), 0, s, pa, p.cand, p.aux);
    if (ksplit > 1 && pa.want_n2) {
        hipLaunchKernelGGL(k_eval_cnorm, dim3((unsigned)(p.ntiles * 16)), dim3(256), 0, s, pa, p.aux);
    }
    }
    const DeviceModel dm = to_device_model(m);
    const unsigned qb = (unsigned)((n + 3) / 4);
#define KGE_Q(MID) case MID: hipLaunchKernelGGL((k_eval_queries<MID>), dim3((MID == KGE_TRANSE || MID == KGE_TRANSH || MID == KGE_TRANSD || MID == KGE_TRANSM) ? qb : (unsigned)n), dim3(256), 0, s, dm, triples, n, p.K, p.Kpad, p.QV, p.qvec, p.qscale, side); break;
    switch (m->model) {
        KGE_Q(KGE_TRANSE) KGE_Q(KGE_TRANSH) KGE_Q(KGE_TRANSD) KGE_Q(KGE_ROTATE) KGE_Q(KGE_DISTMULT)
        KGE_Q(KGE_COMPLEX) KGE_Q(KGE_ANALOGY) KGE_Q(KGE_RESCAL)
        KGE_Q(KGE_TRANSM) KGE_Q(KGE_CP) KGE_Q(KGE_SIMPLE) KGE_Q(KGE_SIMPLE_IGNR) KGE_Q(KGE_QUATE) KGE_Q(KGE_HEAD_1N_INTERNAL) KGE_Q(KGE_DOT_INTERNAL)
        default: set_error("kge_eval: unsupported model %d", m->model); return -1;
    }
#undef KGE_Q
    }
    if (scores_out == nullptr) (void)hipMemsetAsync(p.rcount, 0, (size_t)4 * n * sizeof(int32_t), s);
#define KGE_S(F, X) launch_tf_and_sweep<F, X>(p, m, triples, tail_off, tail_ids, head_off, head_ids, scores_out, s)
    if (p.post == P_SCALE) {
        if (p.form == F_L1) launch_tf_and_sweep<F_L1, X_NONE, P_SCALE>(p, m, triples, tail_off, tail_ids, head_off, head_ids, scores_out, s);
        else launch_tf_and_sweep<F_L2, X_NONE, P_SCALE>(p, m, triples, tail_off, tail_ids, head_off, head_ids, scores_out, s);
    } else if (p.post == P_CLAMP) {
        launch_tf_and_sweep<F_NEGDOT, X_NONE, P_CLAMP>(p, m, triples, tail_off, tail_ids, head_off, head_ids, scores_out, s);
    } else if (p.post == P_SIGMOID) {
        launch_tf_and_sweep<F_NEGDOT, X_NONE, P_SIGMOID>(p, m, triples, tail_off, tail_ids, head_off, head_ids, scores_out, s);
    } else if (p.xform == X_NONE) {
        switch (p.form) {
            case F_L1: KGE_S(F_L1, X_NONE); break;
            case F_L2: KGE_S(F_L2, X_NONE); break;
            case F_SQM: KGE_S(F_SQM, X_NONE); break;
            default: KGE_S(F_NEGDOT, X_NONE); break;
        }
    } else if (p.xform == X_TRANSH) {
        if (p.form == F_L1) KGE_S(F_L1, X_TRANSH); else KGE_S(F_L2, X_TRANSH);
    } else {
        if (p.form == F_L1) KGE_S(F_L1, X_TRANSD); else KGE_S(F_L2, X_TRANSD);
    }
#undef KGE_S
    if (scores_out == nullptr) {
        if (side == 2) hipLaunchKernelGGL(k_eval_finalize, dim3((unsigned)((n + 255) / 256)), dim3(256), 0, s, p.rcount, p.fcount, n, ranks, p.tcount, ties);
        else hipLaunchKernelGGL(k_eval_finalize_side, dim3((unsigned)((n + 255) / 256)), dim3(256), 0, s, p.rcount, p.fcount, n, ranks, p.tcount, ties);
    }
    return check_launch("kge_eval pipeline");
}

int launch_eval_ranks(const kge_model_desc* m, const int64_t* triples, int64_t n, const int64_t* tail_off,
                      const int32_t* tail_ids, const int64_t* head_off, const int32_t* head_ids, void* ws,
                      size_t ws_bytes, int32_t* ranks, int32_t* ties, hipStream_t s) {
    EvalFn* eval = model_ops(m->model)->eval;
    return (eval ? eval : run_pipeline)(m, triples, n, tail_off, tail_ids, head_off, head_ids, ws, ws_bytes, ranks, ties, nullptr, s, 2);
}

int launch_eval_ranks_grouped(const kge_model_desc* m, const int64_t* triples, int64_t n, const int32_t* group_of_triple,
                              const int64_t* group_rel, int64_t n_groups, const int32_t* qblocks, int64_t n_qblocks,
                              const int64_t* tail_off, const int32_t* tail_ids, const int64_t* head_off,
                              const int32_t* head_ids, void* ws, size_t ws_bytes, int32_t* ranks, int32_t* ties, hipStream_t s) {
    if (m->model != KGE_TRANSR && m->model != KGE_TRANSH && m->model != KGE_TRANSD) {
        set_error("kge_eval_ranks_grouped: TransR / TransH / TransD only (the other models' candidates do not depend on the relation)");
        return -1;
    }
    if (n_groups < 1 || n_groups > 65535) { set_error("kge_eval_ranks_grouped: %lld relation groups per call (1..65535)", (long long)n_groups); return -1; }
    EvalPlan p;
    if (!make_plan(m, n, ws, &p, n_groups == 1 ? 2 : n_groups)) { set_error("kge_eval: model %d has no sweep form", m->model); return -1; }
    if (ws == nullptr || ws_bytes < p.bytes) {
        set_error("kge_eval_ranks_grouped: workspace too small (%zu < %zu)", ws_bytes, p.bytes);
        return -1;
    }
    if (m->model == KGE_TRANSR) {
        int rc = launch_transr_eval_prepare(m, triples, n, group_rel, n_groups, p.Kpad, p.ntiles, p.cand, p.qvec, p.qscale, s);
        if (rc) return rc;
    } else {
        XfPrepArgs xa;
        xa.ent = m->tables[0]; xa.group_rel = group_rel; xa.E = p.E; xa.K = p.K; xa.Kpad = p.Kpad; xa.table_stride = p.table_stride;
        xa.xform = m->model == KGE_TRANSH ? X_TRANSH : X_TRANSD;
        xa.vec_tab = m->model == KGE_TRANSH ? m->tables[2] : m->tables[3];
        xa.ent_map = m->model == KGE_TRANSD ? m->tables[2] : nullptr;
        hipLaunchKernelGGL(k_eval_prepare_xf, dim3((unsigned)p.ntiles, (unsigned)n_groups), dim3(256), 0, s, xa, p.cand);
        const DeviceModel dm = to_device_model(m);
        const unsigned qb = (unsigned)((n + 3) / 4);
        if (m->model == KGE_TRANSH)
            hipLaunchKernelGGL((k_eval_queries<KGE_TRANSH>), dim3(qb), dim3(256), 0, s, dm, triples, n, p.K, p.Kpad, p.QV, p.qvec, p.qscale, 2);
        else
            hipLaunchKernelGGL((k_eval_queries<KGE_TRANSD>), dim3(qb), dim3(256), 0, s, dm, triples, n, p.K, p.Kpad, p.QV, p.qvec, p.qscale, 2);
    }
    (void)hipMemsetAsync(p.rcount, 0, (size_t)4 * n * sizeof(int32_t), s);
    if (p.form == F_L1)
        launch_tf_and_sweep<F_L1, X_NONE>(p, m, triples, tail_off, tail_ids, head_off, head_ids, nullptr, s, group_of_triple,
                                          qblocks, n_qblocks);
    else
        launch_tf_and_sweep<F_L2, X_NONE>(p, m, triples, tail_off, tail_ids, head_off, head_ids, nullptr, s, group_of_triple,
                                          qblocks, n_qblocks);
    hipLaunchKernelGGL(k_eval_finalize, dim3((unsigned)((n + 255) / 256)), dim3(256), 0, s, p.rcount, p.fcount, n, ranks, p.tcount, ties);
    return check_launch("kge_eval grouped pipeline");
}

int launch_eval_sweep_scores(const kge_model_desc* m, const int64_t* triples, int64_t n, void* ws, size_t ws_bytes,
                             float* scores, hipStream_t s, int side) {
    EvalFn* eval = model_ops(m->model)->eval;
    return (eval ? eval : run_pipeline)(m, triples, n, nullptr, nullptr, nullptr, nullptr, ws, ws_bytes, nullptr, nullptr, scores, s, side);
}

static kge_model_desc dot_desc(const float* cand, const float* q, int K, int64_t E, bool sigmoid) {
    kge_model_desc m;
    memset(&m, 0, sizeof(m));
    m.model = KGE_DOT_INTERNAL;
    m.flags = sigmoid ? kDotSigmoid : 0u;
    m.tot_entity = E; m.tot_relation = 1; m.dim = K; m.rel_dim = K;
    m.tables[0] = const_cast<float*>(cand); m.tables[2] = const_cast<float*>(q);
    return m;
}

size_t dot_eval_workspace_bytes(int64_t n, int K, int64_t E, bool sigmoid) {
    const kge_model_desc m = dot_desc(nullptr, nullptr, K, E, sigmoid);
    EvalPlan p;
    return make_plan(&m, n, nullptr, &p) ? p.bytes : 0;
}

int launch_dot_eval(const float* cand, const float* q, int K, int64_t E, const int64_t* triples, int64_t n, const int64_t* tail_off,
                    const int32_t* tail_ids, const int64_t* head_off, const int32_t* head_ids, void* ws, size_t ws_bytes,
                    int32_t* ranks, int32_t* ties, float* scores, hipStream_t s, int side, bool sigmoid) {
    const kge_model_desc m = dot_desc(cand, q, K, E, sigmoid);
    return run_pipeline(&m, triples, n, tail_off, tail_ids, head_off, head_ids, ws, ws_bytes, ranks, ties, scores, s, side);
}

DotRowsPlan dot_rows_plan(void* ws, int64_t E, int64_t n, int K, bool sigmoid) {
    DotRowsPlan w;
    size_t off = 0;
    char* base = (char*)ws;
    auto take = [&](size_t b) { char* p = base ? base + off : nullptr; off += align256(b); return p; };
    w.cand = (float*)take((size_t)E * K * 4);
    w.qrows = (float*)take((size_t)2 * n * K * 4);
    w.pipe_bytes = dot_eval_workspace_bytes(n, K, E, sigmoid);
    w.pipe = take(w.pipe_bytes);
    w.bytes = off;
    return w;
}

static kge_model_desc head_rank_desc(const float* x, int dim, const float* ent, int64_t E, const float* bias) {
    kge_model_desc m;
    memset(&m, 0, sizeof(m));
    m.model = KGE_HEAD_1N_INTERNAL;
    m.tot_entity = E; m.tot_relation = 1; m.dim = dim; m.rel_dim = dim;
    m.tables[0] = const_cast<float*>(ent); m.tables[1] = const_cast<float*>(bias); m.tables[2] = const_cast<float*>(x);
    return m;
}

size_t head_rank_workspace_bytes(int64_t n, int dim, int64_t E, bool has_bias) {
    static const float one = 1.0f;
    const kge_model_desc m = head_rank_desc(nullptr, dim, nullptr, E, has_bias ? &one : nullptr);
    EvalPlan p;
    return make_plan(&m, n, nullptr, &p) ? p.bytes : 0;
}

int launch_head_rank(const float* x, int64_t n, int dim, const float* ent, int64_t E, const float* bias, const int64_t* triples,
                     const int64_t* off, const int32_t* ids, void* ws, size_t ws_bytes, int32_t* ranks, int32_t* ties, float* energies,
                     hipStream_t s) {
    const kge_model_desc m = head_rank_desc(x, dim, ent, E, bias);
    return run_pipeline(&m, triples, n, off, ids, nullptr, nullptr, ws, ws_bytes, ranks, ties, energies, s, 0);
}

}
```

### pykg2vec_amd/csrc/kge_internal.h

```cpp
#pragma once
#include <hip/hip_runtime.h>
#include <stdint.h>
#include <stddef.h>
#include "../../include/kge_hip.h"
#include "kge_device.h"

#ifdef KGE_NO_LDS_PREFETCH
#define KGE_KEEP_READS_AHEAD() ((void)0)
#else
#define KGE_KEEP_READS_AHEAD() __builtin_amdgcn_sched_barrier(0)
#endif

namespace kge {

void set_error(const char* fmt, ...);
inline size_t align256(size_t x) { return (x + 255) & ~(size_t)255; }

typedef size_t WsBytesFn(const kge_model_desc* m, int64_t n);
typedef int ScoreFwdFn(const kge_model_desc* m, const int64_t* h, const int64_t* r, const int64_t* t, int64_t n, float* scores,
                       void* ws, size_t ws_bytes, hipStream_t s);
typedef int ScoreBwdFn(const kge_model_desc* m, const int64_t* h, const int64_t* r, const int64_t* t, int64_t n, const float* dscore,
                       void* ws, size_t ws_bytes, hipStream_t s);
typedef int PairFwdFn(const kge_model_desc* m, const int64_t* ph, const int64_t* pr, const int64_t* pt, const int64_t* nh,
                      const int64_t* nr, const int64_t* nt, int64_t n, float* scores2, void* ws, size_t ws_bytes, hipStream_t s);
// ... 122 lines not shown
bool rescal_stage_ok(const kge_model_desc* m, int64_t n, size_t ws_bytes);
int launch_rescal_pair_step(const kge_model_desc* m, const int64_t* ph, const int64_t* pr, const int64_t* pt, const int64_t* nh,
                            const int64_t* nt, int64_t n, float margin, float* loss, void* ws, size_t ws_bytes, unsigned* touched,
                            const kge_rescal_stage* stage , hipStream_t s);

int launch_optimizer(int kind, float* p, float* g, float* s1, float* s2, int64_t numel, float lr, int64_t step,
                     int zero_grad, const float* dev_hyper, const int64_t* cursor_in, int64_t* cursor_out, float* hyper_out,
                     int64_t batch_stride, int64_t n_batches, int64_t draws_per_batch, hipStream_t s);

int launch_optimizer_rows(int kind, float* p, float* g, float* s1, float* s2, int64_t rows, int dim, float lr, int64_t step,
                          int zero_grad, int normalize, const float* dev_hyper, const unsigned* touched, unsigned* touched_clear,
                          const kge_rescal_stage* stage , hipStream_t s);

bool optimizer_rownorm_ok(int64_t rows, int64_t dim, size_t scratch_floats);
int launch_optimizer_rownorm(int kind, float* p, float* g, float* s1, float* s2, int64_t rows, int64_t dim, float lr, int64_t step,
                             int zero_grad, const float* dev_hyper, float* scratch, size_t scratch_floats, const int64_t* cursor_in,
                             int64_t* cursor_out, float* hyper_out, int64_t batch_stride, int64_t n_batches, int64_t draws_per_batch,
                             hipStream_t s);

int launch_optimizer_rows_rownorm(int kind, float* p, float* g, float* s1, float* s2, int64_t rows, int dim, float* wp, float* wg,
                                  float* ws1, float* ws2, int64_t wrows, int64_t wdim, float lr, int64_t step, int zero_grad, int normalize,
                                  const float* dev_hyper, const unsigned* touched, unsigned* touched_clear, const kge_rescal_stage* st,
                                  float* scratch, size_t scratch_floats, const int64_t* cursor_in, int64_t* cursor_out, float* hyper_out,
                                  int64_t batch_stride, int64_t n_batches, int64_t draws_per_batch, hipStream_t s);

int pull_partial_stride(int dim);
int pull_hat_stride(int dim);
bool ownx_model(int model);
int ownx_groups_per_block(int model, int dim);
int ownx_partial_stride(int model, int dim);
size_t ownx_stage_floats(int model, int dim, int64_t n_pairs);
int launch_ownx_step(const kge_model_desc* m, float* const* state1, float* const* state2, const int32_t* pairs, int64_t n_pairs,
                     const kge_pull_lists* lists, const int32_t* items, int64_t n_items, const uint32_t* listed, const int32_t* inc,
                     float* partials, const int32_t* multi, int64_t n_multi, int dense, float lmbda, int reg_type, int optimizer, float lr,
                     int64_t step, const int32_t* next_pairs, const int32_t* next_inv, int64_t next_n, const float* bern,
                     const uint64_t* slots, int64_t n_slots, uint64_t seed, uint64_t next_offset, const kge_pull_lists* next_lists,
                     float* loss, float* stage, hipStream_t s);
int transx_groups_per_block(int dim);
int transx_partial_stride(int dim);
void transx_scratch_bytes(int model, int dim, int64_t n, size_t* stage, size_t* recs);
int launch_transx_grad_step(const kge_model_desc* m, const int32_t* pairs, int64_t n_pairs, const kge_pull_lists* lists,
                            const int32_t* items, int64_t n_items, const uint32_t* listed, const int32_t* inc, float* partials,
                            const int32_t* multi, int64_t n_multi, float margin, float* stage, float* recs, int reset_lists,
                            const int32_t* next_pairs, const int32_t* next_inv, int64_t next_n, const float* bern,
                            const uint64_t* slots, int64_t n_slots, uint64_t seed, uint64_t next_offset,
                            const kge_pull_lists* next_lists, float* loss, hipStream_t s);
void pull_direction_bytes(int dim, int l1, int64_t n, size_t* codes, size_t* recs);
int pull_groups_per_block(int dim);
int launch_pull_step(const kge_model_desc* m, float* const tables_out[2], const float* const hat_in[2], float* const hat_out[2],
                     const float* norm_in, float* norm_out, float* const state1[2], float* const state2[2], const int32_t* pairs,
                     const kge_pull_lists* lists, const int32_t* items, int64_t n_items, const uint32_t* dense_skip, const int32_t* inc, float* partials,
                     const int32_t* multi, int64_t n_multi, float margin, int optimizer, float lr, int64_t step,
                     const float* dev_hyper, int reset_lists, const int32_t* next_pairs, const int32_t* next_inv, int64_t next_n, const float* bern,
                     const uint64_t* slots, int64_t n_slots, uint64_t seed, uint64_t next_offset,
                     const kge_pull_lists* next_lists, float* loss, const kge_pull_direction* dir, hipStream_t s);
int launch_row_norms(const float* table, int64_t rows, int dim, float* out, float* hat, hipStream_t s);
int launch_pull_sample(const int32_t* pairs, const int32_t* inv, int64_t n, int64_t E, const float* bern, const uint64_t* slots, int64_t n_slots,
                       uint64_t seed, uint64_t offset, const int64_t* cursor, const kge_pull_lists* out, hipStream_t s);
int launch_pull_lists_explicit(const int32_t* pairs, const int32_t* inv, const int64_t* nh, const int64_t* nt, int64_t n,
                               const kge_pull_lists* out, hipStream_t s);

int own_groups_per_block(int model, int dim);
int own_partial_stride(int model, int dim);
int launch_own_step(const kge_model_desc* m, const int32_t* pairs, int64_t n_pairs, const kge_pull_lists* lists, const int32_t* items,
                    int64_t n_items, const uint32_t* listed, const int32_t* inc, float* partials, int dense, float lmbda, int reg_type,
                    int reset_lists, const int32_t* next_pairs, const int32_t* next_inv, int64_t next_n, const float* bern,
                    const uint64_t* slots, int64_t n_slots, uint64_t seed, uint64_t next_offset, const kge_pull_lists* next_lists,
                    float* loss, float* stage, hipStream_t s);
int launch_own_apply(const kge_model_desc* m, float* const* state1, float* const* state2, const int32_t* pairs, int64_t n_pairs,
                     const kge_pull_lists* lists, const int32_t* items, int64_t n_items, const uint32_t* listed, const int32_t* multi,
                     int64_t n_multi, float* partials, int dense, int optimizer, float lr, int64_t step, int multi_only, hipStream_t s);
int launch_own_step_fused(const kge_model_desc* m, float* const* state1, float* const* state2, const int32_t* pairs, int64_t n_pairs,
                          const kge_pull_lists* lists, const int32_t* items, int64_t n_items, const uint32_t* listed, const int32_t* inc,
                          float* partials, int dense, float lmbda, int reg_type, int optimizer, float lr, int64_t step,
                          const int32_t* next_pairs, const int32_t* next_inv, int64_t next_n, const float* bern, const uint64_t* slots,
                          int64_t n_slots, uint64_t seed, uint64_t next_offset, const kge_pull_lists* next_lists, float* loss,
                          float* stage, hipStream_t s);

size_t eval_workspace_bytes(const kge_model_desc* m, int64_t n, int64_t tables = 1);
int launch_eval_ranks_grouped(const kge_model_desc* m, const int64_t* triples, int64_t n, const int32_t* group_of_triple,
                              const int64_t* group_rel, int64_t n_groups, const int32_t* qblocks, int64_t n_qblocks,
                              const int64_t* tail_off, const int32_t* tail_ids, const int64_t* head_off,
                              const int32_t* head_ids, void* ws, size_t ws_bytes, int32_t* ranks, int32_t* ties, hipStream_t s);
int launch_eval_ranks(const kge_model_desc* m, const int64_t* triples, int64_t n, const int64_t* tail_off,
                      const int32_t* tail_ids, const int64_t* head_off, const int32_t* head_ids, void* ws,
                      size_t ws_bytes, int32_t* ranks, int32_t* ties , hipStream_t s);
int launch_eval_sweep_scores(const kge_model_desc* m, const int64_t* triples, int64_t n, void* ws, size_t ws_bytes,
                             float* scores, hipStream_t s, int side = 2);
constexpr int KGE_HEAD_1N_INTERNAL = 100;
size_t head_rank_workspace_bytes(int64_t n, int dim, int64_t E, bool has_bias);
int launch_head_rank(const float* x, int64_t n, int dim, const float* ent, int64_t E, const float* bias, const int64_t* triples,
                     const int64_t* off, const int32_t* ids, void* ws, size_t ws_bytes, int32_t* ranks, int32_t* ties, float* energies,
                     hipStream_t s);

int launch_rank_from_scores(const float* scores, int64_t nq, int64_t E, const int64_t* truth, const int64_t* off,
                            const int32_t* ids, int32_t* rank, int32_t* frank, hipStream_t s);

constexpr int KGE_DOT_INTERNAL = 101;
constexpr uint32_t kDotSigmoid = 1u << 8;
size_t dot_eval_workspace_bytes(int64_t n, int K, int64_t E, bool sigmoid = false);
int launch_dot_eval(const float* cand, const float* q, int K, int64_t E, const int64_t* triples, int64_t n, const int64_t* tail_off,
                    const int32_t* tail_ids, const int64_t* head_off, const int32_t* head_ids, void* ws, size_t ws_bytes,
                    int32_t* ranks, int32_t* ties, float* scores, hipStream_t s, int side, bool sigmoid = false);
struct DotRowsPlan { float* cand; float* qrows; void* pipe; size_t pipe_bytes, bytes; };
DotRowsPlan dot_rows_plan(void* ws, int64_t E, int64_t n, int K, bool sigmoid = false);

ScoreFwdFn launch_hole_forward, launch_octonion_forward, launch_semantic_forward;
ScoreBwdFn launch_hole_backward, launch_octonion_backward, launch_semantic_backward;
PairFwdFn launch_hole_pair_forward, launch_semantic_pair_forward;
PairBwdFn launch_hole_pair_backward, launch_semantic_pair_backward;
WsBytesFn semantic_workspace_bytes;
WsBytesFn hole_eval_workspace_bytes, octonion_eval_workspace_bytes, kg2e_eval_workspace_bytes, semantic_eval_workspace_bytes,
          ntn_eval_workspace_bytes;
EvalFn launch_hole_eval, launch_octonion_eval, launch_kg2e_eval, launch_semantic_eval, launch_ntn_eval;
int launch_octonion_pointwise(const kge_model_desc* m, const int64_t* h, const int64_t* r, const int64_t* t, const int64_t* y,
                              int64_t n, int bundle, float lmbda, int reg_type, float* loss, hipStream_t s);
int launch_octonion_pointwise_sampled(const kge_model_desc* m, const int64_t* triples, const int64_t* perm, int64_t start,
                                      int64_t n_pos, int neg_rate, const float* bern, const uint64_t* slots, int64_t n_slots,
                                      uint64_t seed, uint64_t offset, const int64_t* cursor, float lmbda, int reg_type, float* loss,
                                      hipStream_t s);
inline bool is_semantic_model(int model) { return model == KGE_SLM || model == KGE_SME || model == KGE_SME_BL; }

int launch_head_forward(const float* x, int64_t B, int d, const float* ent, int64_t E, const float* bias, float* preds,
                        int bf16, hipStream_t s);
size_t head_backward_workspace_bytes();
int launch_head_backward(const float* x, int64_t B, int d, const float* ent, int64_t E, const float* preds,
                         const float* dpreds, float* dx, float* g_ent, float* g_bias, void* ws, size_t ws_bytes, hipStream_t s);
size_t head_bce_workspace_bytes(int64_t B, int64_t E, int64_t n_pos);
int launch_head_bce(const float* x, int64_t B, int d, const float* ent, int64_t E, const float* bias,
                    const int64_t* lab_off, const int32_t* lab_ids, int64_t n_pos, float label_smoothing, void* ws,
                    size_t ws_bytes, float* loss, float* dx, float* g_ent, float* g_bias, hipStream_t s);

int launch_triple_set_build(const int64_t* triples, int64_t n, uint64_t* slots, int64_t n_slots, hipStream_t s);
int launch_corrupt(const int64_t* ph, const int64_t* pr, const int64_t* pt, int64_t n_pos, int neg_rate,
                   int64_t E, const float* bern, const uint64_t* slots, int64_t n_slots, uint64_t seed,
                   uint64_t offset, int64_t* nh, int64_t* nr, int64_t* nt, hipStream_t s);

int launch_sample_batch(const int64_t* triples, const int64_t* perm, int64_t start, int64_t n_pos, int neg_rate,
                        int64_t E, const float* bern, const uint64_t* slots, int64_t n_slots, uint64_t seed,
                        uint64_t offset, int layout, int64_t* const out[6], const int64_t* cursor, hipStream_t s);
int launch_step_advance(int64_t* cursor, float* hyper, int64_t batch_stride, int64_t n_batches, int64_t draws_per_batch,
                        float lr, hipStream_t s);

inline int check_launch(const char* what) {
    hipError_t e = hipGetLastError();
    if (e != hipSuccess) {
        set_error("%s: %s", what, hipGetErrorString(e));
        return -2;
    }
    return 0;
}

}
```

### pykg2vec_amd/kernels.py

```python
import ctypes
import os
import math

import torch

from . import _lib as L

MODEL_IDS = {"transe": L.TRANSE, "transh": L.TRANSH, "transd": L.TRANSD, "rotate": L.ROTATE, "rescal": L.RESCAL,
             "ntn": L.NTN, "distmult": L.DISTMULT, "complex": L.COMPLEX, "complexn3": L.COMPLEX, "analogy": L.ANALOGY,
             "transm": L.TRANSM, "cp": L.CP, "simple": L.SIMPLE, "simple_ignr": L.SIMPLE_IGNR, "quate": L.QUATE,
             "transr": L.TRANSR, "slm": L.SLM, "sme": L.SME, "sme_bl": L.SME_BL, "kg2e": L.KG2E, "hole": L.HOLE,
             "octonione": L.OCTONIONE}
OPTIMIZER_IDS = {"sgd": L.OPT_SGD, "adam": L.OPT_ADAM, "adagrad": L.OPT_ADAGRAD, "rms": L.OPT_RMSPROP,
                 "gradient": 4}


def _stream():
    return ctypes.c_void_p(torch.cuda.current_stream().cuda_stream)


def _dev(t, dtype, what):
    if not isinstance(t, torch.Tensor):
        raise TypeError("%s must be a tensor" % what)
    if not t.is_cuda:
        raise L.KgeHipError("%s must live on the HIP device (got %s); the HIP path has no CPU fallback" % (what, t.device))
    if t.dtype != dtype:
        raise TypeError("%s must be %s (got %s)" % (what, dtype, t.dtype))
    if not t.is_contiguous():
        raise ValueError("%s must be contiguous" % what)
    return ctypes.c_void_p(t.data_ptr())


def _ids(t, what):
    return _dev(t, torch.int64, what)


_TABLE_SHAPES = {
    "transe": [("E", "d"), ("R", "d")],
    "transm": [("E", "d"), ("R", "d"), ("R", None)],
    "transh": [("E", "d"), ("R", "d"), ("R", "d")],
    "transd": [("E", "d"), ("R", "k"), ("E", "d"), ("R", "k")],
    "rotate": [("E", "d"), ("E", "d"), ("R", "d")],
    "rescal": [("E", "d"), ("R", "d*d")],
    "ntn": [("E", "d"), ("R", "k"), ("d", "k"), ("d", "k"), (1, "k"), ("k", "d*d")],
    "transr": [("E", "d"), ("R", "k"), ("R", "d*k")],
    "slm": [("E", "d"), ("R", "k"), ("d", "k"), ("d", "k")],
    "sme": [("E", "d"), ("R", "d"), ("d", "d"), ("d", "d"), ("d", 1), ("d", "d"), ("d", "d"), ("d", 1)],
    "sme_bl": [("E", "d"), ("R", "d"), ("d", "d"), ("d", "d"), ("d", 1), ("d", "d"), ("d", "d"), ("d", 1)],
    "kg2e": [("E", "d"), ("E", "d"), ("R", "d"), ("R", "d")],
    "hole": [("E", "d"), ("R", "d")],
    "distmult": [("E", "d"), ("R", "d")],
    "complex": [("E", "d"), ("E", "d"), ("R", "d"), ("R", "d")],
    "complexn3": [("E", "d"), ("E", "d"), ("R", "d"), ("R", "d")],
    "analogy": [("E", "d"), ("R", "d"), ("E", "d/2"), ("E", "d/2"), ("R", "d/2"), ("R", "d/2")],
    "cp": [("E", "d"), ("R", "d"), ("E", "d")],
    "simple": [("E", "d"), ("E", "d"), ("R", "d"), ("R", "d")],
    "simple_ignr": [("E", "d"), ("E", "d"), ("R", "d"), ("R", "d")],
    "quate": [("E", "d")] * 4 + [("R", "d")] * 4,
    "octonione": [("E", "d")] * 8 + [("R", "d")] * 8 + [("R", "d")],
}


def _check_table_shapes(model_name, tables, tot_entity, tot_relation, dim, rel_dim):
    spec = _TABLE_SHAPES.get(model_name)
    if spec is None:
        return
    if len(tables) < len(spec):
        raise L.KgeHipError("%s: %d tables given, the model has %d" % (model_name, len(tables), len(spec)))
    size = {"E": int(tot_entity), "R": int(tot_relation), "d": int(dim), "k": int(rel_dim)}
    cols_of = {"d": size["d"], "k": size["k"], "d*d": size["d"] ** 2, "d*k": size["d"] * size["k"], "d/2": size["d"] // 2}
    for i, ((by, cols), t) in enumerate(zip(spec, tables)):
        rows = t.shape[0]
        want_cols = cols_of.get(cols)
        got_cols = t.numel() // rows if rows else 0
        if by in ("E", "R"):
            need = size[by]
            if rows < need:
                raise L.KgeHipError(
                    "%s: table %d has %d rows but is indexed by %s ids up to %d (tot_%s = %d): an nn.Embedding lookup would raise "
                    "IndexError (models/Domain.py:8-13)" % (model_name, i, rows, "entity" if by == "E" else "relation", need - 1,
                                                             "entity" if by == "E" else "relation", need))
        else:
            need = by if isinstance(by, int) else size[by]
            if rows != need:
                raise L.KgeHipError("%s: table %d must have %d rows (got %d)" % (model_name, i, need, rows))
        if want_cols is not None and (t.dim() != 2 or got_cols != want_cols):
            raise L.KgeHipError("%s: table %d must be [rows, %d] (got %s)" % (model_name, i, want_cols, tuple(t.shape)))


def set_debug(check_ids=True):
    L.load().kge_set_debug(1 if check_ids else 0)


def set_switch(name, value):
    L.check(L.load().kge_set_switch(name.encode(), -1 if value is None else int(value)), "kge_set_switch")


def debug_enabled():
    return bool(L.load().kge_get_debug())


def check_ids(ids, bound, what="ids"):
    L.check(L.load().kge_check_ids(_ids(ids, what), ids.numel(), int(bound), _stream()), "kge_check_ids(%s)" % what)


def debug_marker(tag):
    L.check(L.load().kge_debug_marker(int(tag), _stream()), "kge_debug_marker")


def make_desc(model_name, tables, grads=None, *, tot_entity, tot_relation, dim, rel_dim=None, l1_flag=False,
              margin=0.0):
    _check_table_shapes(model_name, tables, tot_entity, tot_relation, dim, rel_dim if rel_dim is not None else dim)
    d = L.ModelDesc()
    d.model = MODEL_IDS[model_name]
    d.flags = L.FLAG_L1 if l1_flag else 0
    d.tot_entity, d.tot_relation = int(tot_entity), int(tot_relation)
    d.dim = int(dim)
    d.rel_dim = int(rel_dim if rel_dim is not None else dim)
    d.margin = float(margin)
    d.phase_scale = 0.0
    if model_name == "rotate":
        d.phase_scale = 1.0 / (((float(margin) + 2.0) / dim) / 3.14159265358979323846)
    for i, t in enumerate(tables):
        d.tables[i] = _dev(t, torch.float32, "table %d" % i).value
    if grads is not None:
        for i, g in enumerate(grads):
            if g.shape != tables[i].shape:
                raise ValueError("grad %d shape %s != table shape %s" % (i, tuple(g.shape), tuple(tables[i].shape)))
            d.grads[i] = _dev(g, torch.float32, "grad %d" % i).value
    d._keepalive = (tables, grads)
    return d


def _block_of(tensors, rows, dim):
    stride = (rows * dim + 3) // 4 * 4 * 4
    t0 = tensors[0]
    for c, t in enumerate(tensors):
        if not (t.is_cuda and t.dtype == torch.float32 and t.is_contiguous() and tuple(t.shape) == (rows, dim)
                and t.device == t0.device and t.data_ptr() == t0.data_ptr() + c * stride):
            return None
    return t0


def _pack_block(tensors, rows, dim):
    stride = (rows * dim + 3) // 4 * 4
    for i, t in enumerate(tensors):
        _dev(t, torch.float32, "table %d" % i)
    blk = torch.zeros(len(tensors) * stride, dtype=torch.float32, device=tensors[0].device)
    for c, t in enumerate(tensors):
        blk[c * stride:c * stride + rows * dim].view(rows, dim).copy_(t[:rows])
    return blk


def octonion_desc(tables, grads=None, *, tot_entity, tot_relation, dim):
    _check_table_shapes("octonione", tables, tot_entity, tot_relation, dim, dim)
    E, R, d = int(tot_entity), int(tot_relation), int(dim)
    desc = L.ModelDesc()
    desc.model = L.OCTONIONE
    desc.flags = 0
    desc.tot_entity, desc.tot_relation = E, R
    desc.dim = desc.rel_dim = d
    desc.margin = desc.phase_scale = 0.0
    keep, after = [], []
    for slot, (lo, rows) in enumerate(((0, E), (8, R))):
        parts = list(tables[lo:lo + 8])
        blk = _block_of(parts, rows, d)
        if blk is None:
            blk = _pack_block(parts, rows, d)
        desc.tables[slot] = blk.data_ptr()
        keep.append(blk)
        if grads is not None:
            gparts = list(grads[lo:lo + 8])
            for g, t in zip(gparts, parts):
                if g.shape != t.shape:
                    raise ValueError("grad shape %s != table shape %s" % (tuple(g.shape), tuple(t.shape)))
            gblk = _block_of(gparts, rows, d)
            if gblk is None:
                gblk = _pack_block(gparts, rows, d)
# ... 414 lines not shown
    L.check(lib.kge_optimizer_step_rownorm(OPTIMIZER_IDS[kind], _dev(param, torch.float32, "param"), _dev(grad, torch.float32, "grad"), p1, p2,
                                           int(rows), int(dim), float(lr), int(step), 1 if zero_grad else 0, adv[0], sc.data_ptr(), sc.numel() * 4,
                                           adv[1], adv[2], adv[3], adv[4], adv[5], adv[6], _stream()), "kge_optimizer_step_rownorm")


def optimizer_step_rows_rownorm(kind, param, grad, state1, state2, rows, dim, wparam, wgrad, wstate1, wstate2, wrows, wdim, lr, step,
                                normalize=True, dev_hyper=None, touched=None, touched_clear=None, stage=None, advance=None, zero_grad=True):
    lib = L.load()
    need = 4 * int(wrows) * ((int(wdim) + 4095) // 4096)
    key = (param.device, "rider", need)
    if key not in _rescal_scratch:
        _rescal_scratch[key] = torch.empty(max(1, need // 4), dtype=torch.float32, device=param.device)
    sc = _rescal_scratch[key]
    f = lambda t, what: _dev(t, torch.float32, what) if t is not None else None
    if advance is not None:
        hyper, cursor, next_cursor, next_hyper, batch_stride, n_batches, draws = advance
        adv = (_dev(cursor, torch.int64, "cursor"), _dev(next_cursor, torch.int64, "next_cursor"), _dev(next_hyper, torch.float32, "next_hyper"),
               int(batch_stride), int(n_batches), int(draws))
        dev_hyper = hyper
    else:
        adv = (None, None, None, 0, 1, 0)
    L.check(lib.kge_optimizer_step_rows_rownorm(
        OPTIMIZER_IDS[kind], _dev(param, torch.float32, "param"), _dev(grad, torch.float32, "grad"), f(state1, "state1"), f(state2, "state2"),
        int(rows), int(dim), _dev(wparam, torch.float32, "wparam"), _dev(wgrad, torch.float32, "wgrad"), f(wstate1, "wstate1"),
        f(wstate2, "wstate2"), int(wrows), int(wdim), float(lr), int(step), 1 if zero_grad else 0, 1 if normalize else 0, f(dev_hyper, "dev_hyper"),
        _dev(touched, torch.int32, "touched") if touched is not None else None,
        _dev(touched_clear, torch.int32, "touched_clear") if touched_clear is not None else None,
        ctypes.byref(stage.c) if stage is not None else None, sc.data_ptr(), sc.numel() * 4, adv[0], adv[1], adv[2], adv[3], adv[4], adv[5],
        _stream()), "kge_optimizer_step_rows_rownorm")


def optimizer_step_advance(kind, param, grad, state1, state2, lr, hyper, cursor, next_cursor, next_hyper, batch_stride,
                           n_batches, draws_per_batch, zero_grad=True):
    p1 = _dev(state1, torch.float32, "state1") if state1 is not None else None
    p2 = _dev(state2, torch.float32, "state2") if state2 is not None else None
    L.check(L.load().kge_optimizer_step_advance(
        OPTIMIZER_IDS[kind], _dev(param, torch.float32, "param"), _dev(grad, torch.float32, "grad"), p1, p2, param.numel(),
        float(lr), 1 if zero_grad else 0, _dev(hyper, torch.float32, "hyper"), _dev(cursor, torch.int64, "cursor"),
        _dev(next_cursor, torch.int64, "next_cursor"), _dev(next_hyper, torch.float32, "next_hyper"), int(batch_stride),
        int(n_batches), int(draws_per_batch), _stream()), "kge_optimizer_step_advance")


def step_advance(cursor, hyper, batch_stride, n_batches, draws_per_batch, lr):
    L.check(L.load().kge_step_advance(_dev(cursor, torch.int64, "cursor"), _dev(hyper, torch.float32, "hyper"),
                                      int(batch_stride), int(n_batches), int(draws_per_batch), float(lr), _stream()),
            "kge_step_advance")


def eval_workspace(desc, n, device):
    nbytes = L.load().kge_eval_workspace_bytes(ctypes.byref(desc), int(n))
    if nbytes == 0:
        L.check(-1, "kge_eval_workspace_bytes")
    return torch.empty(nbytes, dtype=torch.uint8, device=device)


def eval_ranks(desc, triples, tail_off, tail_ids, head_off, head_ids, workspace=None, ties=None):
    if isinstance(desc, L.MurpDesc):
        return murp_eval_ranks(desc, triples, tail_off, tail_ids, head_off, head_ids, ties=ties)
    if isinstance(desc, L.ConvKBDesc):
        if ties is not None:
            ties.fill_(-1)
        return convkb_eval_ranks(desc, triples, tail_off, tail_ids, head_off, head_ids)
    if isinstance(desc, L.TuckerDesc):
        return tucker_eval_ranks(desc, triples, tail_off, tail_ids, head_off, head_ids, ties=ties)
    if isinstance(desc, L.ProjeDesc):
        return proje_eval_ranks(desc, triples, tail_off, tail_ids, head_off, head_ids, ties=ties)
    if isinstance(desc, L.ConveDesc):
        return conve_eval_ranks(desc, triples, tail_off, tail_ids, head_off, head_ids, ties=ties)
    if isinstance(desc, L.HyperDesc):
        return hyper_eval_ranks(desc, triples, tail_off, tail_ids, head_off, head_ids, ties=ties)
    if isinstance(desc, L.InteracteDesc):
        return interacte_eval_ranks(desc, triples, tail_off, tail_ids, head_off, head_ids, ties=ties)
    if isinstance(desc, L.AcreDesc):
        return acre_eval_ranks(desc, triples, tail_off, tail_ids, head_off, head_ids, ties=ties)
    n = triples.shape[0]
    if workspace is None:
        workspace = eval_workspace(desc, n, triples.device)
    ranks = torch.empty((4, n), dtype=torch.int32, device=triples.device)
    args = _filter_csr_args(tail_off, tail_ids, head_off, head_ids)
    L.check(L.load().kge_eval_ranks_ties(ctypes.byref(desc), _ids(triples, "triples"), n, *args,
                                         _dev(workspace, torch.uint8, "workspace"), workspace.numel(),
                                         _dev(ranks, torch.int32, "ranks"),
                                         _dev(ties, torch.int32, "ties") if ties is not None else None, _stream()), "kge_eval_ranks")
    return ranks


def eval_ranks_grouped(desc, triples, group_of_triple, group_rel, qblocks, tail_off, tail_ids, head_off, head_ids, ties=None):
    n, G = triples.shape[0], group_rel.shape[0]
    lib = L.load()
    nbytes = lib.kge_eval_grouped_workspace_bytes(ctypes.byref(desc), int(n), int(G))
    if nbytes == 0:
        L.check(-1, "kge_eval_grouped_workspace_bytes")
    workspace = torch.empty(nbytes, dtype=torch.uint8, device=triples.device)
    ranks = torch.empty((4, n), dtype=torch.int32, device=triples.device)
    args = _filter_csr_args(tail_off, tail_ids, head_off, head_ids)
    L.check(lib.kge_eval_ranks_grouped_ties(ctypes.byref(desc), _ids(triples, "triples"), n,
                                            _dev(group_of_triple, torch.int32, "group_of_triple"), _ids(group_rel, "group_rel"), G,
                                            _dev(qblocks, torch.int32, "qblocks"), qblocks.shape[0], *args,
                                            _dev(workspace, torch.uint8, "workspace"), workspace.numel(),
                                            _dev(ranks, torch.int32, "ranks"),
                                            _dev(ties, torch.int32, "ties") if ties is not None else None, _stream()), "kge_eval_ranks_grouped")
    return ranks


def eval_sweep_scores(desc, triples, workspace=None):
    if isinstance(desc, L.MurpDesc):
        both = torch.stack([murp_sweep_scores_side(desc, triples, 0), murp_sweep_scores_side(desc, triples, 1)], 1)
        return both.view(2 * triples.shape[0], desc.tot_entity)
    if isinstance(desc, L.ConvKBDesc):
        both = torch.stack([convkb_sweep_scores_side(desc, triples, 0), convkb_sweep_scores_side(desc, triples, 1)], 1)
        return both.view(2 * triples.shape[0], desc.tot_entity)
    n = triples.shape[0]
    if workspace is None:
        workspace = eval_workspace(desc, n, triples.device)
    out = torch.empty((2 * n, desc.tot_entity), dtype=torch.float32, device=triples.device)
    L.check(L.load().kge_eval_sweep_scores(ctypes.byref(desc), _ids(triples, "triples"), n,
                                           _dev(workspace, torch.uint8, "workspace"), workspace.numel(),
                                           _dev(out, torch.float32, "scores"), _stream()), "kge_eval_sweep_scores")
    return out


def eval_sweep_scores_side(desc, triples, side, workspace=None):
    if isinstance(desc, L.MurpDesc):
        return murp_sweep_scores_side(desc, triples, side)
    if isinstance(desc, L.ConvKBDesc):
        return convkb_sweep_scores_side(desc, triples, side)
    if desc.model in (MODEL_IDS["transr"], MODEL_IDS["ntn"], MODEL_IDS["slm"]):
        return eval_sweep_scores(desc, triples, workspace)[int(side)::2]
    n = triples.shape[0]
    if workspace is None:
        workspace = eval_workspace(desc, n, triples.device)
    out = torch.empty((n, desc.tot_entity), dtype=torch.float32, device=triples.device)
    L.check(L.load().kge_eval_sweep_scores_side(ctypes.byref(desc), _ids(triples, "triples"), n, int(side),
                                                _dev(workspace, torch.uint8, "workspace"), workspace.numel(),
                                                _dev(out, torch.float32, "scores"), _stream()), "kge_eval_sweep_scores_side")
    return out


def rank_from_scores(scores, truth, off, ids):
    nq, E = scores.shape
    rank = torch.empty(nq, dtype=torch.int32, device=scores.device)
    frank = torch.empty_like(rank)
    po = _dev(off, torch.int64, "csr offsets") if off is not None else None
    pi = _dev(ids, torch.int32, "csr ids") if ids is not None else None
    L.check(L.load().kge_rank_from_scores(_dev(scores, torch.float32, "scores"), nq, E, _ids(truth, "truth"), po, pi,
                                          _dev(rank, torch.int32, "rank"), _dev(frank, torch.int32, "frank"), _stream()),
            "kge_rank_from_scores")
    return rank, frank


def eval_ranks_via_forward(desc, triples, tail_off, tail_ids, head_off, head_ids, chunk=64):
    n = triples.shape[0]
    E = desc.tot_entity
    dev = triples.device
    ents = torch.arange(E, dtype=torch.int64, device=dev)
    out = torch.empty((4, n), dtype=torch.int32, device=dev)
    for lo in range(0, n, chunk):
        tr = triples[lo:lo + chunk]
        m = tr.shape[0]
        h, r, t = tr[:, 0:1], tr[:, 1:2], tr[:, 2:3]
        cand = ents.view(1, E).expand(m, E)
        tail_scores = score_forward(desc, h.expand(m, E).reshape(-1).contiguous(), r.expand(m, E).reshape(-1).contiguous(),
                                    cand.reshape(-1).contiguous()).view(m, E)
        head_scores = score_forward(desc, cand.reshape(-1).contiguous(), r.expand(m, E).reshape(-1).contiguous(),
                                    t.expand(m, E).reshape(-1).contiguous()).view(m, E)
        to = (tail_off[lo:lo + m + 1]).contiguous() if tail_off is not None else None
# ... 1263 lines not shown
```

Measured before the change: 2.652 billion.

## Add quantized 16-bit SAD bound filter for L1 eval ranking with exact fallback

For L1-distance models such as TransE, candidate and query embeddings are quantized to 16-bit fixed point and scored with packed sum-of-absolute-difference instructions. Per-query thresholds then settle most candidates as definitely better or definitely worse than the true triple. Only ambiguous (query, entity) pairs go to a worklist that an exact fp32 kernel rescores, and the original fp32 sweep is skipped unless the bound path signals a fallback. This replaces most of the fp32 work in the ranking sweep, at the cost of extra quantization passes, workspace memory, atomics for the worklist, and a new per-side eval entry point plus stats API.

```diff
diff --git a/include/kge_hip.h b/include/kge_hip.h
--- a/include/kge_hip.h
+++ b/include/kge_hip.h
@@ -60,6 +60,7 @@
 
 int kge_set_debug(int32_t check_ids);
 int kge_set_switch(const char* name, int32_t value);
+int kge_eval_l1b_stats(int32_t* out5, void* stream);
 int kge_get_debug(void);
 int kge_check_ids(const int64_t* ids, int64_t n, int64_t bound, void* stream);
 size_t kge_filter_csr_workspace_bytes(int64_t n_known, int64_t n_queries);
@@ -194,6 +195,8 @@
 int kge_eval_ranks_ties(const kge_model_desc* m, const int64_t* triples, int64_t n, const int64_t* tail_off,
                         const int32_t* tail_ids, const int64_t* head_off, const int32_t* head_ids, void* workspace,
                         size_t workspace_bytes, int32_t* ranks, int32_t* ties, void* stream);
+int kge_eval_ranks_side(const kge_model_desc* m, const int64_t* triples, int64_t n, int side, const int64_t* off, const int32_t* ids,
+                        void* workspace, size_t workspace_bytes, int32_t* ranks, int32_t* ties, void* stream);
 int kge_eval_ranks_grouped_ties(const kge_model_desc* m, const int64_t* triples, int64_t n, const int32_t* group_of_triple,
                                 const int64_t* group_rel, int64_t n_groups, const int32_t* qblocks, int64_t n_qblocks,
                                 const int64_t* tail_off, const int32_t* tail_ids, const int64_t* head_off,
diff --git a/pykg2vec_amd/_lib.py b/pykg2vec_amd/_lib.py
--- a/pykg2vec_amd/_lib.py
+++ b/pykg2vec_amd/_lib.py
@@ -303,6 +303,7 @@
     "kge_abi_version": (ctypes.c_int, []),
     "kge_set_debug": (ctypes.c_int, [ctypes.c_int32]),
     "kge_set_switch": (ctypes.c_int, [ctypes.c_char_p, ctypes.c_int32]),
+    "kge_eval_l1b_stats": (ctypes.c_int, [ctypes.c_void_p, ctypes.c_void_p]),
     "kge_get_debug": (ctypes.c_int, []),
     "kge_check_ids": (ctypes.c_int, [ctypes.c_void_p, ctypes.c_int64, ctypes.c_int64, ctypes.c_void_p]),
     "kge_debug_marker": (ctypes.c_int, [ctypes.c_int32, ctypes.c_void_p]),
@@ -386,6 +387,8 @@
     "kge_eval_workspace_bytes": (ctypes.c_size_t, [ctypes.POINTER(ModelDesc), ctypes.c_int64]),
     "kge_eval_ranks": (ctypes.c_int, [ctypes.POINTER(ModelDesc), ctypes.c_void_p, ctypes.c_int64] + [ctypes.c_void_p] * 4 + [ctypes.c_void_p, ctypes.c_size_t, ctypes.c_void_p, ctypes.c_void_p]),
     "kge_eval_ranks_ties": (ctypes.c_int, [ctypes.POINTER(ModelDesc), ctypes.c_void_p, ctypes.c_int64] + [ctypes.c_void_p] * 4 + [ctypes.c_void_p, ctypes.c_size_t, ctypes.c_void_p, ctypes.c_void_p, ctypes.c_void_p]),
+    "kge_eval_ranks_side": (ctypes.c_int, [ctypes.POINTER(ModelDesc), ctypes.c_void_p, ctypes.c_int64, ctypes.c_int, ctypes.c_void_p,
+                                           ctypes.c_void_p, ctypes.c_void_p, ctypes.c_size_t, ctypes.c_void_p, ctypes.c_void_p, ctypes.c_void_p]),
     "kge_eval_ranks_grouped_ties": (ctypes.c_int, [ctypes.POINTER(ModelDesc), ctypes.c_void_p, ctypes.c_int64, ctypes.c_void_p,
                                                    ctypes.c_void_p, ctypes.c_int64, ctypes.c_void_p, ctypes.c_int64]
                                     + [ctypes.c_void_p] * 4 + [ctypes.c_void_p, ctypes.c_size_t, ctypes.c_void_p, ctypes.c_void_p, ctypes.c_void_p]),
diff --git a/pykg2vec_amd/csrc/kge_api.hip b/pykg2vec_amd/csrc/kge_api.hip
--- a/pykg2vec_amd/csrc/kge_api.hip
+++ b/pykg2vec_amd/csrc/kge_api.hip
@@ -818,6 +818,22 @@
                              (hipStream_t)stream);
 }
 
+int kge_eval_ranks_side(const kge_model_desc* m, const int64_t* triples, int64_t n, int side, const int64_t* off, const int32_t* ids,
+                        void* workspace, size_t workspace_bytes, int32_t* ranks, int32_t* ties, void* stream) {
+    if (validate(m, false, "kge_eval_ranks_side")) return -1;
+    if (n == 0) return 0;
+    if (n < 0 || !triples || !ranks || (side != 0 && side != 1) || (off && !ids)) {
+        set_error("kge_eval_ranks_side: bad arguments (side is 0 = tail sweep or 1 = head sweep)");
+        return -1;
+    }
+    if (m->model == KGE_TRANSR || m->model == KGE_NTN || m->model == KGE_SLM) {
+        set_error("kge_eval_ranks_side: TransR / NTN / SLM compute both sides per call (kge_eval_ranks)");
+        return -1;
+    }
+    if (int rc = debug_check_triples("kge_eval_ranks_side", m->tot_entity, m->tot_relation, triples, n, (hipStream_t)stream)) return rc;
+    return launch_eval_ranks_side(m, triples, n, side, off, ids, workspace, workspace_bytes, ranks, ties, (hipStream_t)stream);
+}
+
 int kge_eval_ranks(const kge_model_desc* m, const int64_t* triples, int64_t n, const int64_t* tail_off,
                    const int32_t* tail_ids, const int64_t* head_off, const int32_t* head_ids, void* workspace,
                    size_t workspace_bytes, int32_t* ranks, void* stream) {
diff --git a/pykg2vec_amd/csrc/kge_debug.hip b/pykg2vec_amd/csrc/kge_debug.hip
--- a/pykg2vec_amd/csrc/kge_debug.hip
+++ b/pykg2vec_amd/csrc/kge_debug.hip
@@ -6,7 +6,7 @@
 namespace kge {
 
 struct SwitchOverride { char name[32]; int value; };
-static SwitchOverride g_overrides[16];
+static SwitchOverride g_overrides[32];
 static int g_n_overrides = 0;
 
 int switch_value(const char* name) {
@@ -21,7 +21,7 @@
 static int set_switch(const char* name, int value) {
     for (int i = 0; i < g_n_overrides; ++i)
         if (!strcmp(g_overrides[i].name, name)) { g_overrides[i].value = value; return 0; }
-    if (g_n_overrides == 16 || strlen(name) >= sizeof(g_overrides[0].name)) return -1;
+    if (g_n_overrides == 32 || strlen(name) >= sizeof(g_overrides[0].name)) return -1;
     strcpy(g_overrides[g_n_overrides].name, name);
     g_overrides[g_n_overrides++].value = value;
     return 0;
diff --git a/pykg2vec_amd/csrc/kge_eval.hip b/pykg2vec_amd/csrc/kge_eval.hip
--- a/pykg2vec_amd/csrc/kge_eval.hip
+++ b/pykg2vec_amd/csrc/kge_eval.hip
@@ -1,4 +1,5 @@
 #include "kge_internal.h"
+#include "kge_l1_bound.h"
 #include <stdlib.h>
 #include <string.h>
 
@@ -24,8 +25,18 @@
     int64_t ntiles;
     float* cand; float* aux; float* qvec; float* qscale; float* st; int32_t* fcount; int32_t* rcount; int32_t* tcount;
     float* qT;
+    int32_t* l1b_state;
+    int32_t* rcount_b;
+    uint32_t* c16;
+    float* crow;
+    uint32_t* q16;
+    int32_t* thr;
+    uint2* wl;
+    int64_t wl_cap;
     size_t bytes;
 };
+constexpr int kL1bState = 64;
+constexpr int kL1bChunk = 64;
 
 static int sweep_K(const kge_model_desc* m) {
     switch (m->model) {
@@ -73,6 +84,21 @@
     p->qT = nullptr;
     if ((p->form == F_NEGDOT || p->form == F_SQM) && p->xform == X_NONE)
         p->qT = (float*)take((size_t)((2 * n + 127) / 128) * p->Kpad * 128 * sizeof(float));
+    p->l1b_state = nullptr; p->rcount_b = nullptr; p->c16 = nullptr; p->crow = nullptr; p->q16 = nullptr; p->thr = nullptr; p->wl = nullptr;
+    p->wl_cap = 0;
+    if (p->form == F_L1 && p->xform == X_NONE && p->post == P_NONE && tables == 1 && p->Kpad <= kL1bMaxKpad && p->E < (1ll << 31) &&
+        2 * n < (1ll << 31)) {
+        int64_t cap = (2 * n * p->E / 128 + 4096 + kL1bChunk - 1) / kL1bChunk * kL1bChunk;
+        if (cap > (1ll << 30)) cap = 1ll << 30;
+        p->wl_cap = cap;
+        p->l1b_state = (int32_t*)take(((size_t)kL1bState + 4 * n) * sizeof(int32_t));
+        p->rcount_b = p->l1b_state ? p->l1b_state + kL1bState : nullptr;
+        p->c16 = (uint32_t*)take((size_t)p->ntiles * (p->Kpad / 2) * 64 * sizeof(uint32_t));
+        p->crow = (float*)take((size_t)p->ntiles * 64 * p->Kpad * sizeof(float));
+        p->q16 = (uint32_t*)take((size_t)2 * n * (p->Kpad / 2) * sizeof(uint32_t));
+        p->thr = (int32_t*)take((size_t)4 * n * sizeof(int32_t));
+        p->wl = (uint2*)take((size_t)cap * sizeof(uint2));
+    }
     p->bytes = off;
     return true;
 }
@@ -838,7 +864,9 @@
                                                     int64_t nq, int64_t E, int64_t ntiles, int Kpad, int QV, float margin,
                                                     int S, int qblocks, int32_t* __restrict__ rcount,
                                                     int32_t* __restrict__ tcount, float* __restrict__ scores_out,
-                                                    const int32_t* __restrict__ qdesc, int64_t table_stride) {
+                                                    const int32_t* __restrict__ qdesc, int64_t table_stride,
+                                                    const int32_t* __restrict__ l1b_state) {
+    if (l1b_state != nullptr && l1b_state[1] == 0) return;
     const int lane = threadIdx.x & 63;
     const int wave = threadIdx.x >> 6;
     const int slot = blockIdx.x & 255;
@@ -1007,6 +1035,191 @@
             }
         }
     }
+}
+
+__global__ __launch_bounds__(256) void k_l1b_absmax(const float* __restrict__ cand, int64_t ncand, int64_t E, int Kpad,
+                                                    const float* __restrict__ qvec, int64_t nqel, int32_t* __restrict__ state) {
+    uint32_t m = 0;
+    const int64_t stride = (int64_t)gridDim.x * blockDim.x, i0 = (int64_t)blockIdx.x * blockDim.x + threadIdx.x;
+    const int64_t tile_el = (int64_t)Kpad * 64;
+    for (int64_t i = i0; i < ncand; i += stride)
+        if ((i / tile_el) * 64 + (i & 63) < E) m = max(m, __float_as_uint(cand[i]) & 0x7fffffffu);
+    for (int64_t i = i0; i < nqel; i += stride) m = max(m, __float_as_uint(qvec[i]) & 0x7fffffffu);
+#pragma unroll
+    for (int o = 32; o > 0; o >>= 1) m = max(m, (uint32_t)__shfl_xor((int)m, o, 64));
+    if ((threadIdx.x & 63) == 0 && m != 0) atomicMax((uint32_t*)state, m);
+}
+
+__global__ __launch_bounds__(256) void k_l1b_quant(const float* __restrict__ cand, int64_t ncpair, int Kpad, const float* __restrict__ qvec,
+                                                   int64_t nqpair, int32_t* __restrict__ state, uint32_t* __restrict__ c16,
+                                                   float* __restrict__ crow, uint32_t* __restrict__ q16) {
+    const float M = __uint_as_float((uint32_t)state[0]);
+    const int64_t i = (int64_t)blockIdx.x * blockDim.x + threadIdx.x;
+    if (!l1b_grid_ok(M)) { if (i == 0) state[1] = 1; return; }
+    const double g = l1b_scale(M);
+    const int Kp2 = Kpad / 2;
+    if (i < ncpair) {
+        const int lane = (int)(i & 63);
+        const int64_t r = i >> 6, tile = r / Kp2;
+        const int kp = (int)(r - tile * Kp2);
+        const float c0 = cand[(tile * Kpad + 2 * kp) * 64 + lane], c1 = cand[(tile * Kpad + 2 * kp + 1) * 64 + lane];
+        c16[i] = l1b_pack(l1b_quant(c0, M, g), l1b_quant(c1, M, g));
+        *reinterpret_cast<float2*>(crow + (tile * 64 + lane) * Kpad + 2 * kp) = make_float2(c0, c1);
+    } else if (i - ncpair < nqpair) {
+        const float2 v = reinterpret_cast<const float2*>(qvec)[i - ncpair];
+        q16[i - ncpair] = l1b_pack(l1b_quant(v.x, M, g), l1b_quant(v.y, M, g));
+    }
+}
+
+__global__ __launch_bounds__(256) void k_l1b_thresholds(const float* __restrict__ st, int64_t nq, int Kpad, int32_t* __restrict__ state,
+                                                        int32_t* __restrict__ thr) {
+    const int64_t q = (int64_t)blockIdx.x * blockDim.x + threadIdx.x;
+    if (q >= nq || state[1] != 0) return;
+    const float s = st[q];
+    if (!(s >= 0.f) || s > 3.0e38f) { atomicOr(&state[1], 1); return; }
+    int32_t A, B;
+    l1b_thresholds(s, l1b_scale(__uint_as_float((uint32_t)state[0])), Kpad, &A, &B);
+    thr[2 * q] = A; thr[2 * q + 1] = B;
+}
+
+constexpr int KC2 = KC / 2;
+template <int QT, class F>
+__device__ __forceinline__ void for_query_chunks_u32(const uint32_t* const (&qrow)[QT], int off, F body) {
+    uint32_t nx[KC2];
+#pragma unroll
+    for (int j = 0; j < KC2; ++j) nx[j] = qrow[0][off + j];
+#pragma unroll
+    for (int q = 0; q < QT; ++q) {
+        uint32_t cur[KC2];
+#pragma unroll
+        for (int j = 0; j < KC2; ++j) cur[j] = nx[j];
+        asm volatile("" ::"s"(cur[0]), "s"(cur[KC2 - 1]));
+        if (q + 1 < QT) {
+#pragma unroll
+            for (int j = 0; j < KC2; ++j) nx[j] = qrow[q + 1][off + j];
+        }
+        __builtin_amdgcn_sched_barrier(0);
+        body(q, cur);
+        __builtin_amdgcn_sched_barrier(0);
+    }
+}
+
+template <int QT>
+__global__ __launch_bounds__(256) void k_eval_sweep_l1b(const uint32_t* __restrict__ c16, const uint32_t* __restrict__ q16,
+                                                        const int32_t* __restrict__ thr, int64_t nq, int64_t E, int64_t ntiles, int Kp2,
+                                                        int S, int qblocks, int32_t* __restrict__ rcount_b, uint2* __restrict__ wl,
+                                                        int wl_cap, int32_t* __restrict__ state) {
+    if (state[1] != 0) return;
+    const int lane = threadIdx.x & 63;
+    const int wave = threadIdx.x >> 6;
+    const int slot = blockIdx.x & 255;
+    const int mm = blockIdx.x >> 8;
+    const int ts = mm % S;
+    const int qb = (mm / S) * 256 + slot;
+    if (qb >= qblocks) return;
+    const int64_t q0 = (int64_t)qb * QT;
+    const uint32_t* qrow[QT];
+    int cnt[QT];
+#pragma unroll
+    for (int q = 0; q < QT; ++q) {
+        const int64_t qi = (q0 + q < nq) ? q0 + q : nq - 1;
+        qrow[q] = q16 + qi * Kp2;
+        cnt[q] = 0;
+    }
+    int wl_pos = 0, wl_end = 0, n_real = 0;
+    bool dead = false;
+    auto append = [&](uint64_t mask, uint32_t qidx, uint32_t e) {
+        const int m = __popcll(mask);
+        if (wl_pos + m > wl_end) {
+            if (wl_pos + lane < wl_end) wl[wl_pos + lane] = make_uint2(0xffffffffu, 0u);
+            int base = 0;
+            if (lane == 0) base = atomicAdd(&state[2], kL1bChunk);
+            base = __builtin_amdgcn_readfirstlane(base);
+            if (base < 0 || base > wl_cap - kL1bChunk) {
+                if (lane == 0) atomicOr(&state[1], 1);
+                dead = true; wl_pos = 0; wl_end = 0;
+                return;
+            }
+            wl_pos = base; wl_end = base + kL1bChunk;
+        }
+        if ((mask >> lane) & 1) {
+            const int rank = __builtin_amdgcn_mbcnt_hi((uint32_t)(mask >> 32), __builtin_amdgcn_mbcnt_lo((uint32_t)mask, 0u));
+            wl[wl_pos + rank] = make_uint2(qidx, e);
+        }
+        wl_pos += m; n_real += m;
+    };
+    for (int64_t tile = ((int64_t)ts * 4 + wave) * 2; tile < ntiles; tile += (int64_t)S * 8) {
+        const bool has_b = tile + 1 < ntiles;
+        const uint32_t* ca = c16 + (tile * Kp2) * 64 + lane;
+        const uint32_t* cb = has_b ? ca + (int64_t)Kp2 * 64 : ca;
+        uint32_t acca[QT], accb[QT];
+#pragma unroll
+        for (int q = 0; q < QT; ++q) { acca[q] = 0u; accb[q] = 0u; }
+        for (int k0 = 0; k0 < Kp2; k0 += KC2) {
+            uint32_t va[KC2], vb[KC2];
+#pragma unroll
+            for (int j = 0; j < KC2; ++j) { va[j] = ca[(int64_t)(k0 + j) * 64]; vb[j] = cb[(int64_t)(k0 + j) * 64]; }
+            for_query_chunks_u32<QT>(qrow, k0, [&](int q, const uint32_t (&qv)[KC2]) {
+#pragma unroll
+                for (int j = 0; j < KC2; ++j) {
+                    acca[q] = __builtin_amdgcn_sad_u16(va[j], qv[j], acca[q]);
+                    accb[q] = __builtin_amdgcn_sad_u16(vb[j], qv[j], accb[q]);
+                }
+            });
+        }
+        const int64_t ea = tile * 64 + lane, eb = ea + 64;
+        const bool valid_a = ea < E, valid_b = has_b && eb < E;
+#pragma unroll
+        for (int q = 0; q < QT; ++q) {
+            const int64_t qi = (q0 + q < nq) ? q0 + q : nq - 1;
+            const int A = thr[2 * qi], B = thr[2 * qi + 1];
+            const int ia = (int)acca[q], ib = (int)accb[q];
+            cnt[q] += __popcll(__ballot(valid_a && ia <= A)) + __popcll(__ballot(valid_b && ib <= A));
+            if (q0 + q < nq && !dead) {
+                const uint64_t ma = __ballot(valid_a && ia > A && ia < B);
+                if (ma != 0) append(ma, (uint32_t)qi, (uint32_t)ea);
+                const uint64_t mb = __ballot(valid_b && ib > A && ib < B);
+                if (mb != 0 && !dead) append(mb, (uint32_t)qi, (uint32_t)eb);
+            }
+        }
+    }
+    if (wl_pos + lane < wl_end) wl[wl_pos + lane] = make_uint2(0xffffffffu, 0u);
+    if (lane == 0) {
+#pragma unroll
+        for (int q = 0; q < QT; ++q)
+            if (q0 + q < nq && cnt[q] != 0) atomicAdd(rcount_b + q0 + q, cnt[q]);
+        if (n_real != 0) atomicAdd(&state[3], n_real);
+    }
+}
+
+__device__ __forceinline__ float l1_row_score(const float* __restrict__ c, const float* __restrict__ q, int Kpad) {
+    float acc = 0.f;
+    for (int k0 = 0; k0 < Kpad; k0 += KC) {
+        float cv[KC], qv[KC];
+#pragma unroll
+        for (int j = 0; j < KC; j += 4) {
+            *reinterpret_cast<float4*>(cv + j) = *reinterpret_cast<const float4*>(c + k0 + j);
+            *reinterpret_cast<float4*>(qv + j) = *reinterpret_cast<const float4*>(q + k0 + j);
+        }
+#pragma unroll
+        for (int j = 0; j < KC; ++j) acc = pair_step<F_L1>(acc, cv[j], qv[j]);
+    }
+    return pair_post<P_NONE>(pair_finish<F_L1>(acc, 0.f), 1.0f);
+}
+
+__global__ __launch_bounds__(256) void k_eval_l1b_exact(const uint2* __restrict__ wl, const int32_t* __restrict__ state, int wl_cap,
+                                                        const float* __restrict__ crow, const float* __restrict__ qvec,
+                                                        const float* __restrict__ st, int Kpad, int32_t* __restrict__ rcount_b,
+                                                        int32_t* __restrict__ tcount_b) {
+    if (state[1] != 0) return;
+    const int64_t i = (int64_t)blockIdx.x * blockDim.x + threadIdx.x;
+    if (i >= min(state[2], wl_cap)) return;
+    const uint2 ent = wl[i];
+    if (ent.x == 0xffffffffu) return;
+    const float s = l1_row_score(crow + (int64_t)ent.y * Kpad, qvec + (int64_t)ent.x * Kpad, Kpad);
+    const float t = st[ent.x];
+    if (s < t) atomicAdd(rcount_b + ent.x, 1);
+    else if (s == t) atomicAdd(tcount_b + ent.x, 1);
 }
 
 typedef float f32x16 __attribute__((ext_vector_type(16)));
@@ -1339,7 +1552,9 @@
 #endif
 
 __global__ void k_eval_finalize(const int32_t* __restrict__ rcount, const int32_t* __restrict__ fcount, int64_t n,
-                                int32_t* __restrict__ ranks, const int32_t* __restrict__ tcount, int32_t* __restrict__ ties) {
+                                int32_t* __restrict__ ranks, const int32_t* __restrict__ tcount, int32_t* __restrict__ ties,
+                                const int32_t* __restrict__ l1b_state = nullptr, const int32_t* __restrict__ rcount_b = nullptr) {
+    if (l1b_state != nullptr && l1b_state[1] == 0) { rcount = rcount_b; tcount = rcount_b + 2 * n; }
     const int64_t i = (int64_t)blockIdx.x * blockDim.x + threadIdx.x;
     if (i >= n) return;
     if (ties) {
@@ -1354,7 +1569,9 @@
 }
 
 __global__ void k_eval_finalize_side(const int32_t* __restrict__ rcount, const int32_t* __restrict__ fcount, int64_t n,
-                                     int32_t* __restrict__ ranks, const int32_t* __restrict__ tcount, int32_t* __restrict__ ties) {
+                                     int32_t* __restrict__ ranks, const int32_t* __restrict__ tcount, int32_t* __restrict__ ties,
+                                     const int32_t* __restrict__ l1b_state = nullptr, const int32_t* __restrict__ rcount_b = nullptr) {
+    if (l1b_state != nullptr && l1b_state[1] == 0) { rcount = rcount_b; tcount = rcount_b + 2 * n; }
     const int64_t i = (int64_t)blockIdx.x * blockDim.x + threadIdx.x;
     if (i >= n) return;
     if (ties) ties[i] = max(0, tcount[i] - 1);
@@ -1425,6 +1642,13 @@
     if (force >= 0) return force == 1;
     return nq >= 512 && p.Kpad >= 32;
 }
+
+static bool use_l1_bound(const EvalPlan& p, const float* scores_out, const int32_t* group_of_triple, const int32_t* qdesc) {
+    return p.form == F_L1 && p.xform == X_NONE && p.post == P_NONE && scores_out == nullptr && group_of_triple == nullptr &&
+           qdesc == nullptr && p.wl != nullptr && switch_value("EVAL_L1_BOUND") != 0;
+}
+static int32_t* g_l1b_last_state = nullptr;
+static int g_l1b_last_cap = 0;
 
 template <int FORM, int XFORM, int POST = P_NONE>
 static void launch_tf_and_sweep(const EvalPlan& p, const kge_model_desc* m, const int64_t* triples,
@@ -1475,14 +1699,38 @@
         hipLaunchKernelGGL((k_eval_target_filter<FORM, XFORM, POST>), dim3((unsigned)((nq + 3) / 4)), dim3(256), 0, s, p.cand,
                            p.aux, p.qvec, p.qscale, triples, p.n, p.Kpad, p.QV, m->margin, tail_off, tail_ids, head_off, head_ids,
                            p.st, p.fcount, group_of_triple, p.table_stride, p.only);
+    const int32_t* l1b_gate = nullptr;
+    if constexpr (FORM == F_L1 && XFORM == X_NONE && POST == P_NONE) {
+        if (use_l1_bound(p, scores_out, group_of_triple, qdesc)) {
+            const int Kp2 = p.Kpad / 2;
+            const int64_t ncand = p.ntiles * p.Kpad * 64, nqel = nq * p.Kpad;
+            int cap = (int)p.wl_cap;
+            const int cap_sw = switch_value("EVAL_L1_BOUND_CAP");
+            if (cap_sw >= 1 && cap_sw < cap) cap = cap_sw;
+            (void)hipMemsetAsync(p.l1b_state, 0, ((size_t)kL1bState + 4 * p.n) * sizeof(int32_t), s);
+            const int64_t nel = ncand + nqel;
+            hipLaunchKernelGGL(k_l1b_absmax, dim3((unsigned)min((int64_t)2048, (nel + 255) / 256)), dim3(256), 0, s, p.cand, ncand, p.E,
+                               p.Kpad, p.qvec, nqel, p.l1b_state);
+            hipLaunchKernelGGL(k_l1b_quant, dim3((unsigned)((nel / 2 + 255) / 256)), dim3(256), 0, s, p.cand, ncand / 2, p.Kpad, p.qvec,
+                               nqel / 2, p.l1b_state, p.c16, p.crow, p.q16);
+            hipLaunchKernelGGL(k_l1b_thresholds, dim3((unsigned)((nq + 255) / 256)), dim3(256), 0, s, p.st, nq, p.Kpad, p.l1b_state, p.thr);
+            hipLaunchKernelGGL((k_eval_sweep_l1b<QT>), dim3(grid), dim3(256), 0, s, p.c16, p.q16, p.thr, nq, p.E, p.ntiles, Kp2, (int)S,
+                               qblocks, p.rcount_b, p.wl, cap, p.l1b_state);
+            hipLaunchKernelGGL(k_eval_l1b_exact, dim3((unsigned)((cap + 255) / 256)), dim3(256), 0, s, p.wl, p.l1b_state, cap, p.crow,
+                               p.qvec, p.st, p.Kpad, p.rcount_b, p.rcount_b + 2 * p.n);
+            l1b_gate = p.l1b_state;
+            g_l1b_last_state = p.l1b_state;
+            g_l1b_last_cap = cap;
+        }
+    }
     if (scores_out == nullptr) {
         hipLaunchKernelGGL((k_eval_sweep<FORM, XFORM, QT, false, POST>), dim3(grid), dim3(256), 0, s, p.cand, p.aux, p.qvec,
                            p.qscale, p.st, nq, p.E, p.ntiles, p.Kpad, p.QV, m->margin, (int)S, qblocks, p.rcount, p.tcount, nullptr,
-                           qdesc, p.table_stride);
+                           qdesc, p.table_stride, l1b_gate);
     } else {
         hipLaunchKernelGGL((k_eval_sweep<FORM, XFORM, QT, true, POST>), dim3(grid), dim3(256), 0, s, p.cand, p.aux, p.qvec,
                            p.qscale, p.st, nq, p.E, p.ntiles, p.Kpad, p.QV, m->margin, (int)S, qblocks, p.rcount, nullptr, scores_out,
-                           qdesc, p.table_stride);
+                           qdesc, p.table_stride, (const int32_t*)nullptr);
     }
 }
 
@@ -1504,6 +1752,7 @@
         return -1;
     }
     if (n <= 0) return 0;
+    g_l1b_last_state = nullptr;
     if (m->model == KGE_TRANSR) {
         int rc = launch_transr_eval_prepare(m, triples, n, nullptr, 1, p.Kpad, p.ntiles, p.cand, p.qvec, p.qscale, s);
         if (rc) return rc;
@@ -1575,8 +1824,9 @@
     }
 #undef KGE_S
     if (scores_out == nullptr) {
-        if (side == 2) hipLaunchKernelGGL(k_eval_finalize, dim3((unsigned)((n + 255) / 256)), dim3(256), 0, s, p.rcount, p.fcount, n, ranks, p.tcount, ties);
-        else hipLaunchKernelGGL(k_eval_finalize_side, dim3((unsigned)((n + 255) / 256)), dim3(256), 0, s, p.rcount, p.fcount, n, ranks, p.tcount, ties);
+        const int32_t* l1b = use_l1_bound(p, scores_out, nullptr, nullptr) ? p.l1b_state : nullptr;
+        if (side == 2) hipLaunchKernelGGL(k_eval_finalize, dim3((unsigned)((n + 255) / 256)), dim3(256), 0, s, p.rcount, p.fcount, n, ranks, p.tcount, ties, l1b, (const int32_t*)p.rcount_b);
+        else hipLaunchKernelGGL(k_eval_finalize_side, dim3((unsigned)((n + 255) / 256)), dim3(256), 0, s, p.rcount, p.fcount, n, ranks, p.tcount, ties, l1b, (const int32_t*)p.rcount_b);
     }
     return check_launch("kge_eval pipeline");
 }
@@ -1586,6 +1836,13 @@
                       size_t ws_bytes, int32_t* ranks, int32_t* ties, hipStream_t s) {
     EvalFn* eval = model_ops(m->model)->eval;
     return (eval ? eval : run_pipeline)(m, triples, n, tail_off, tail_ids, head_off, head_ids, ws, ws_bytes, ranks, ties, nullptr, s, 2);
+}
+
+int launch_eval_ranks_side(const kge_model_desc* m, const int64_t* triples, int64_t n, int side, const int64_t* off, const int32_t* ids,
+                           void* ws, size_t ws_bytes, int32_t* ranks, int32_t* ties, hipStream_t s) {
+    if (model_ops(m->model)->eval) { set_error("kge_eval_ranks_side: model %d ranks through a pass of its own (kge_eval_ranks)", m->model); return -1; }
+    return run_pipeline(m, triples, n, side == 0 ? off : nullptr, side == 0 ? ids : nullptr, side == 1 ? off : nullptr,
+                        side == 1 ? ids : nullptr, ws, ws_bytes, ranks, ties, nullptr, s, side);
 }
 
 int launch_eval_ranks_grouped(const kge_model_desc* m, const int64_t* triples, int64_t n, const int32_t* group_of_triple,
@@ -1627,7 +1884,8 @@
     else
         launch_tf_and_sweep<F_L2, X_NONE>(p, m, triples, tail_off, tail_ids, head_off, head_ids, nullptr, s, group_of_triple,
                                           qblocks, n_qblocks);
-    hipLaunchKernelGGL(k_eval_finalize, dim3((unsigned)((n + 255) / 256)), dim3(256), 0, s, p.rcount, p.fcount, n, ranks, p.tcount, ties);
+    hipLaunchKernelGGL(k_eval_finalize, dim3((unsigned)((n + 255) / 256)), dim3(256), 0, s, p.rcount, p.fcount, n, ranks, p.tcount, ties,
+                       (const int32_t*)nullptr, (const int32_t*)nullptr);
     return check_launch("kge_eval grouped pipeline");
 }
 
@@ -1697,3 +1955,16 @@
 }
 
 }
+
+extern "C" int kge_eval_l1b_stats(int32_t* out5, void* stream) {
+    for (int i = 0; i < 5; ++i) out5[i] = 0;
+    if (kge::g_l1b_last_state == nullptr) return 0;
+    int32_t h[4];
+    if (hipMemcpyAsync(h, kge::g_l1b_last_state, sizeof(h), hipMemcpyDeviceToHost, (hipStream_t)stream) != hipSuccess ||
+        hipStreamSynchronize((hipStream_t)stream) != hipSuccess) {
+        kge::set_error("kge_eval_l1b_stats: %s", hipGetErrorString(hipGetLastError()));
+        return -2;
+    }
+    out5[0] = 1; out5[1] = h[1]; out5[2] = h[3]; out5[3] = h[2]; out5[4] = kge::g_l1b_last_cap;
+    return 0;
+}
diff --git a/pykg2vec_amd/csrc/kge_internal.h b/pykg2vec_amd/csrc/kge_internal.h
--- a/pykg2vec_amd/csrc/kge_internal.h
+++ b/pykg2vec_amd/csrc/kge_internal.h
@@ -228,6 +228,8 @@
                               const int64_t* group_rel, int64_t n_groups, const int32_t* qblocks, int64_t n_qblocks,
                               const int64_t* tail_off, const int32_t* tail_ids, const int64_t* head_off,
                               const int32_t* head_ids, void* ws, size_t ws_bytes, int32_t* ranks, int32_t* ties, hipStream_t s);
+int launch_eval_ranks_side(const kge_model_desc* m, const int64_t* triples, int64_t n, int side, const int64_t* off, const int32_t* ids,
+                           void* ws, size_t ws_bytes, int32_t* ranks, int32_t* ties, hipStream_t s);
 int launch_eval_ranks(const kge_model_desc* m, const int64_t* triples, int64_t n, const int64_t* tail_off,
                       const int32_t* tail_ids, const int64_t* head_off, const int32_t* head_ids, void* ws,
                       size_t ws_bytes, int32_t* ranks, int32_t* ties , hipStream_t s);
diff --git a/pykg2vec_amd/csrc/kge_l1_bound.h b/pykg2vec_amd/csrc/kge_l1_bound.h
--- /dev/null
+++ b/pykg2vec_amd/csrc/kge_l1_bound.h
@@ -0,0 +1,44 @@
+#pragma once
+#include <math.h>
+#include <stdint.h>
+
+#if defined(__HIPCC__) || defined(__CUDACC__)
+#define KGE_L1B_HD __host__ __device__ inline
+#else
+#define KGE_L1B_HD inline
+#endif
+
+namespace kge {
+
+constexpr int kL1bMaxKpad = 16384;
+
+KGE_L1B_HD bool l1b_grid_ok(float M) { return M >= 0x1p-100f && M <= 0x1p100f; }
+
+KGE_L1B_HD double l1b_scale(float M) { return 65535.0 / (2.0 * (double)M); }
+
+KGE_L1B_HD uint32_t l1b_quant(float x, float M, double g) {
+    double t = rint(((double)x + (double)M) * g);
+    t = t >= 0.0 ? (t > 65535.0 ? 65535.0 : t) : 0.0;
+    return (uint32_t)t;
+}
+
+KGE_L1B_HD uint32_t l1b_pack(uint32_t lo, uint32_t hi) { return lo | (hi << 16); }
+
+KGE_L1B_HD uint32_t l1b_sad(uint32_t c, uint32_t q, uint32_t acc) {
+    const int32_t dl = (int32_t)(c & 0xffffu) - (int32_t)(q & 0xffffu), dh = (int32_t)(c >> 16) - (int32_t)(q >> 16);
+    return acc + (uint32_t)(dl < 0 ? -dl : dl) + (uint32_t)(dh < 0 ? -dh : dh);
+}
+
+KGE_L1B_HD void l1b_thresholds(float st, double g, int Kpad, int32_t* A, int32_t* B) {
+    const double nu = (double)(Kpad + 1) * 0x1p-24;
+    const double gam = nu / (1.0 - nu);
+    const double x = (double)st * g;
+    double a = floor(x / (1.0 + gam) - (double)(Kpad + 1)) - 1.0;
+    double b = ceil(x / (1.0 - gam) + (double)(Kpad + 1)) + 1.0;
+    a = a < -1.0 ? -1.0 : a > 2147483000.0 ? 2147483000.0 : a;
+    b = b < 0.0 ? 0.0 : b > 2147483600.0 ? 2147483600.0 : b;
+    *A = (int32_t)a;
+    *B = (int32_t)b;
+}
+
+}
diff --git a/pykg2vec_amd/kernels.py b/pykg2vec_amd/kernels.py
--- a/pykg2vec_amd/kernels.py
+++ b/pykg2vec_amd/kernels.py
@@ -94,6 +94,12 @@
 
 def set_switch(name, value):
     L.check(L.load().kge_set_switch(name.encode(), -1 if value is None else int(value)), "kge_set_switch")
+
+
+def eval_l1b_stats():
+    out = (ctypes.c_int32 * 5)()
+    L.check(L.load().kge_eval_l1b_stats(ctypes.cast(out, ctypes.c_void_p), _stream()), "kge_eval_l1b_stats")
+    return dict(zip(("taken", "fallback", "entries", "slots", "capacity"), (int(v) for v in out)))
 
 
 def debug_enabled():
@@ -674,6 +680,19 @@
                                          _dev(workspace, torch.uint8, "workspace"), workspace.numel(),
                                          _dev(ranks, torch.int32, "ranks"),
                                          _dev(ties, torch.int32, "ties") if ties is not None else None, _stream()), "kge_eval_ranks")
+    return ranks
+
+
+def eval_ranks_side(desc, triples, side, off=None, ids=None, workspace=None, ties=None):
+    n = triples.shape[0]
+    if workspace is None:
+        workspace = eval_workspace(desc, n, triples.device)
+    ranks = torch.empty((2, n), dtype=torch.int32, device=triples.device)
+    L.check(L.load().kge_eval_ranks_side(ctypes.byref(desc), _ids(triples, "triples"), n, int(side),
+                                         _dev(off, torch.int64, "csr offsets") if off is not None else None,
+                                         _dev(ids, torch.int32, "csr ids") if ids is not None else None,
+                                         _dev(workspace, torch.uint8, "workspace"), workspace.numel(), _dev(ranks, torch.int32, "ranks"),
+                                         _dev(ties, torch.int32, "ties") if ties is not None else None, _stream()), "kge_eval_ranks_side")
     return ranks
 
 
```

Measured after the change: 2.651 billion. No clear change (-0.0%).
